# EugenHotaj/pytorch-generative

Measured on AMD Instinct MI355X. Metric: training images/sec (ImageGPT 8-block/4-head/16-embed, 28x28x1), higher is better.
Workload: dtype f32; 1 GPU; BASELINE.json configs[1]: ImageGPT 8 blocks / 4 heads / 16 embed on 28x28x1 binarised-MNIST-shaped synthetic; one step = zero_grad + fwd + BCE + bwd + global grad-norm + Adam + lr decay (reference trainer.py:173-193); per_gpu_batch=1024, global_batch=1024, parallelism=dp1, launch=hipGraph replay

## Files before the change

### include/pg_hip.h

```cpp
#ifndef PG_HIP_H_
#define PG_HIP_H_

#include <stddef.h>
#include <stdint.h>

#ifdef __cplusplus
extern "C" {
#endif

#define PG_ABI_VERSION 2

#define PG_EINVAL (-1)
#define PG_ESHAPE (-2)

#define PG_MAX_TAPS 64

#define PG_ACT_NONE 0
#define PG_ACT_RELU 1
#define PG_ACT_ELU 2
#define PG_ACT_GELU 3
#define PG_ACT_ELU_OUT 4

#define PG_GATE_TANH 0
#define PG_GATE_IDENTITY 1

int pg_abi_version(void);
const char* pg_last_error(void);

int pg_conv2d_taps(const float* in, const float* wpk, const float* bias, const float* res,
                   float* out, int N, int Cin, int IH, int IW, int Cout, int OH, int OW,
                   int T, const int* tap_dr, const int* tap_dc, int in_act,
                   const float* dact_src, int dact, void* stream);

int pg_pack_conv_weight(const float* w, float* wpk, int Cout, int Cin, int KH, int KW, int T,
                        const int* tap_u, const int* tap_v, int transpose, int b_pad,
                        void* stream);
size_t pg_packed_weight_floats(int a, int T, int b);
int pg_conv_b_pad(int b);

int pg_conv2d_mfma(const float* in, const float* wfrag, const float* bias, const float* res,
                   float* out, int N, int Cin, int IH, int IW, int Cout, int OH, int OW, int T,
                   const int* tap_dr, const int* tap_dc, int in_act, const float* dact_src,
                   int dact, int out_act, int fmt, void* stream);
int pg_conv2d_mfma_ex(const float* in, const float* wfrag, const float* bias, const float* res,
                      float* out, int N, int Cin, int IH, int IW, int Cout, int OH, int OW, int T,
                      const int* tap_dr, const int* tap_dc, int in_act, const float* dact_src,
                      int dact, int out_act, int fmt, const float* res2, long res_bs, long res2_bs,
                      void* stream);
int pg_conv_gate_fusable(int Cin, int Cout, int OH, int OW, int T, const int* tap_dr, const int* tap_dc);
int pg_conv2d_mfma_gate(const float* in, const float* wfrag, const float* bias, const float* res, float* out, int N, int Cin,
                        int IH, int IW, int Cout, int OH, int OW, int T, const int* tap_dr, const int* tap_dc, int in_act, int gate,
                        const float* gate_res, float* gate_out, void* stream);
int pg_conv_dual_ok(int Cin, int Cout, int OH, int OW);
int pg_conv2d_mfma_dual(const float* in, const float* wfrag, float* out, float* out2, int N, int Cin, int OH, int OW, int Cout,
                        const float* dact_src, int dact, const float* r, void* stream);
#define PG_CONV_FMT_F32 1
#define PG_CONV_FMT_B3 2
#define PG_CONV_FMT_B3_GATE 3
int pg_conv_mfma_supported(int Cin, int Cout, int T, int OH, int OW, int IW, int hr, int hc);
size_t pg_conv_frag_floats(int K_channels, int M_channels, int T, int fmt);
int pg_pack_conv_weight_frag(const float* w, float* wfrag, int Cout, int Cin, int KH, int KW,
                             int T, const int* tap_u, const int* tap_v, int transpose, int fmt,
                             void* stream);
int pg_pack_conv_weight_frag2(const float* w, float* wfrag_fwd, float* wfrag_dgrad, int Cout,
                              int Cin, int KH, int KW, int T, const int* tap_u, const int* tap_v,
                              int fmt_fwd, int fmt_dgrad, void* stream);

int pg_conv2d_wgrad(const float* x, const float* dy, float* dw, float* db, int N, int Cin,
                    int IH, int IW, int Cout, int OH, int OW, int KH, int KW, int T,
                    const int* tap_dr, const int* tap_dc, const int* tap_u, const int* tap_v,
                    int in_act, float* workspace, size_t workspace_floats, void* stream);
size_t pg_conv2d_wgrad_workspace_floats(int Cout, int Cin, int T);

int pg_mul_inplace(float* w, const float* mask, size_t n, void* stream);

int pg_nchw_layernorm_fwd(const float* x, const float* gamma, const float* beta, float* y,
                          float* mean, float* rstd, int N, int C, int L, float eps,
                          void* stream);
int pg_nchw_layernorm_bwd(const float* x, const float* gamma, const float* mean,
                          const float* rstd, const float* dy, float* dx, float* dgamma,
                          float* dbeta, int N, int C, int L, float* workspace,
                          size_t workspace_floats, void* stream);
size_t pg_nchw_layernorm_bwd_workspace_floats(int N, int C, int L);
int pg_nchw_layernorm_bwd_res(const float* x, const float* gamma, const float* mean,
                              const float* rstd, const float* dy, const float* dx_add, float* dx,
                              float* dgamma, float* dbeta, int N, int C, int L, float* workspace,
                              size_t workspace_floats, void* stream);

int pg_causal_attn_fwd(const float* q, const float* k, const float* v, float* o, float* lse2,
                       int N, int heads, int L, int dk, int dv, long q_bs, long k_bs, long v_bs,
                       long o_bs, int strict, void* stream);
int pg_causal_attn_bwd(const float* q, const float* k, const float* v, const float* o,
                       const float* d_o, const float* lse2, float* delta, float* dq, float* dk,
                       float* dv, int N, int heads, int L, int dk_dim, int dv_dim, long q_bs,
                       long k_bs, long v_bs, long o_bs, long do_bs, long dq_bs, long dk_bs,
                       long dv_bs, int strict, void* stream);

int pg_causal_attn_bwd_dq(const float* q, const float* k, const float* v, const float* o,
                          const float* d_o, const float* lse2, float* delta, float* dq, float* dk,
                          float* dv, int N, int heads, int L, int dk_dim, int dv_dim, long q_bs,
                          long k_bs, long v_bs, long o_bs, long do_bs, long dq_bs, long dk_bs,
                          long dv_bs, int strict, void* stream);
int pg_causal_attn_bwd_dkv(const float* q, const float* k, const float* v, const float* o,
                           const float* d_o, const float* lse2, float* delta, float* dq, float* dk,
                           float* dv, int N, int heads, int L, int dk_dim, int dv_dim, long q_bs,
                           long k_bs, long v_bs, long o_bs, long do_bs, long dq_bs, long dk_bs,
                           long dv_bs, int strict, void* stream);

int pg_attn_fused_bwd(int enable);

int pg_attn_block_plan(int which, int L, int waves, int* out_blk, int* out_q0, int* out_ngrp, int* out_wave,
                       int* out_cost);

#define PG_FEATURE_IDENTITY 0
#define PG_FEATURE_ELU1 1
size_t pg_linear_attn_workspace_floats(int N, int heads, int L, int dk, int dv, int backward);
int pg_linear_attn_fwd(const float* q, const float* k, const float* v, float* out, float* den, float* ws,
                       size_t ws_floats, int N, int heads, int L, int dk, int dv, long q_bs, long kv_bs,
                       long o_bs, int feature, void* stream);
int pg_linear_attn_bwd(const float* q, const float* k, const float* v, const float* out, const float* den,
                       const float* g, float* dq, float* dk, float* dv, float* ws, size_t ws_floats, int N,
                       int heads, int L, int dk_dim, int dv_dim, long q_bs, long kv_bs, long o_bs, int feature,
                       void* stream);

size_t pg_masked_linear_workspace_floats(int N, int in, int out, int dgrad);
int pg_masked_linear_fwd(const float* x, float* w, const float* b, const int* deg_in, const int* deg_out, int strict,
                         float* y, int N, int in, int out, int relu, float* ws, size_t ws_floats, void* stream);
int pg_masked_linear_dgrad(const float* dy, const float* w, const int* deg_in, const int* deg_out, int strict,
                           const float* relu_out, float* dx, int N, int in, int out, float* ws, size_t ws_floats,
                           void* stream);
int pg_masked_linear_wgrad(const float* x, const float* dy, float* dw, float* db, int N, int in, int out,
                           void* stream);
int pg_masked_linear_mask(float* mask, const int* deg_in, const int* deg_out, int strict, int in, int out,
                          void* stream);

#define PG_MIXTURE_BERNOULLI 0
#define PG_MIXTURE_GAUSSIAN 1
size_t pg_mixture_workspace_floats(int kind, int N, int K, int F, int backward);
int pg_mixture_fwd(int kind, const float* x, const float* mixture_logits, const float* p1, const float* p2, float* lse,
                   float* stats, int N, int K, int F, float* ws, size_t ws_floats, void* stream);
int pg_mixture_bwd(int kind, const float* x, const float* mixture_logits, const float* p1, const float* p2,
                   const float* stats, const float* g, float* d_logits, float* d1, float* d2, int N, int K, int F,
                   float* ws, size_t ws_floats, void* stream);
size_t pg_kde_workspace_floats(int N, int K, int F);
int pg_kde_gaussian(const float* test, const float* train, float bandwidth, float* out, int N, int K, int F, float* ws,
                    size_t ws_floats, void* stream);
int pg_kde_parzen(const float* test, const float* train, float bandwidth, float coef, float* out, int N, int K, int F,
                  void* stream);

int pg_image_positional_encoding(float* out, int N, int H, int W, void* stream);

int pg_act_fwd(const float* x, float* y, size_t n, int act, void* stream);
int pg_act_bwd(const float* x, const float* dy, float* dx, size_t n, int act, void* stream);
int pg_gated_fwd(const float* x, float* y, int N, int C, int L, int gate, void* stream);
int pg_gated_bwd(const float* x, const float* dy, float* dx, int N, int C, int L, int gate,
                 void* stream);
int pg_gated_fwd_res(const float* x, const float* res, float* y, int N, int C, int L, int gate,
                     void* stream);
int pg_act_bwd_from_out(const float* y, const float* res, const float* dy, float* dx, size_t n,
                        int act, void* stream);
int pg_add(const float* a, const float* b, float* out, size_t n, void* stream);
int pg_fill(float* out, float value, size_t n, void* stream);
int pg_sum_rows(const float* const* rows, const long* batch_strides, int n_rows, float* out, long n_batch, long per, void* stream);
int pg_add_bcast_fwd(const float* x, const float* p, float* y, int N, size_t per, void* stream);
int pg_add_bcast_bwd(const float* dy, float* dp, int N, size_t per, void* stream);

int pg_bce_logits_fwd(const float* z, const float* x, float* loss, int N, size_t per,
                      void* stream);
int pg_bce_logits_bwd(const float* z, const float* x, const float* gscale, float* dz, int N,
                      size_t per, void* stream);

int pg_avgpool2_fwd(const float* x, float* y, int planes, int OH, int OW, void* stream);
int pg_avgpool2_bwd(const float* dy, float* dx, int planes, int OH, int OW, void* stream);
int pg_avgpool2_bwd_res(const float* dy, const float* res, float* dx, int planes, int OH, int OW, void* stream);
int pg_upsample2_fwd(const float* x, float* y, int planes, int IH, int IW, void* stream);
int pg_upsample2_bwd(const float* dy, float* dx, int planes, int IH, int IW, void* stream);
int pg_phase_split2(float* x, float* xs, int planes, int H, int W, int merge, void* stream);
int pg_phase_merge4(float* x, float* const* p, int planes, int H, int W, int merge, void* stream);
int pg_phase_weights(const float* w, float* out, int A, int B, int transposed, void* stream);
int pg_phase_weights_bwd(const float* const* g, float* dw, int A, int B, int transposed, int accumulate, void* stream);
int pg_gauss_head_fwd(const float* q, const float* p, const float* eps, float* z, float* kl, int N,
                      int C, int L, long q_bs, long p_bs, int mode, void* stream);
int pg_gauss_head_bwd(const float* q, const float* p, const float* eps, const float* dz,
                      const float* dkl, float* dq, float* dp, int N, int C, int L, long q_bs,
                      long p_bs, int mode, void* stream);
int pg_vec_mean_accum(const float* v, int n, float* out, void* stream);
int pg_fill_scaled(const float* g, float scale, float* out, int n, void* stream);

int pg_mlp_gelu_fwd(const float* x, const float* w1, const float* b1, const float* w2,
                    const float* b2, const float* res, float* y, int N, int C, int Hd, int L,
                    void* stream);
int pg_mlp_gelu_bwd(const float* x, const float* w1, const float* b1, const float* w2,
                    const float* dy, float* dx, float* dw1, float* db1, float* dw2, float* db2,
                    int N, int C, int Hd, int L, float* workspace, size_t workspace_floats,
                    void* stream);
size_t pg_mlp_gelu_bwd_workspace_floats(int N, int L);

int pg_gpt_block_head_fwd(const float* x, const float* ln_w, const float* ln_b, const float* wq,
                          const float* bq, const float* wkv, const float* bkv, float* qkv, int N,
                          int C, int L, float eps, void* stream);
int pg_gpt_block_head_bwd(const float* x, const float* ln_w, const float* ln_b, const float* wq,
                          const float* wkv, const float* dqkv, const float* gx, float* dx,
                          float* dln_w, float* dln_b, float* dwq, float* dbq, float* dwkv,
                          float* dbkv, int N, int C, int L, float eps, float* workspace,
                          size_t workspace_floats, void* stream);
size_t pg_gpt_block_head_bwd_workspace_floats(int N, int L);
int pg_gpt_block_tail_fwd(const float* o, const float* x, const float* wp, const float* bp,
                          const float* ln_w, const float* ln_b, const float* w1, const float* b1,
                          const float* w2, const float* b2, float* x_new, int N, int C, int Hd,
                          int L, float eps, void* stream);
int pg_gpt_block_tail_bwd(const float* o, const float* x, const float* wp, const float* bp,
                          const float* ln_w, const float* ln_b, const float* w1, const float* b1,
                          const float* w2, const float* dx_new, float* d_o, float* gx, float* dwp,
                          float* dbp, float* dln_w, float* dln_b, float* dw1, float* db1,
                          float* dw2, float* db2, int N, int C, int Hd, int L, float eps,
                          float* workspace, size_t workspace_floats, void* stream);
size_t pg_gpt_block_tail_bwd_workspace_floats(int N, int L);
int pg_gpt_block_tail_bwd_partial(const float* o, const float* x, const float* wp, const float* bp,
                                  const float* ln_w, const float* ln_b, const float* w1, const float* b1,
                                  const float* w2, const float* dx_new, float* d_o, float* gx, int N, int Cc,
                                  int Hd, int L, float eps, float* workspace, size_t workspace_floats,
                                  void* stream);
int pg_gpt_block_head_bwd_with_tail(const float* x, const float* ln_w, const float* ln_b, const float* wq,
                                    const float* wkv, const float* dqkv, const float* gx, float* dx,
                                    float* dln_w, float* dln_b, float* dwq, float* dbq, float* dwkv,
                                    float* dbkv, int N, int Cc, int L, float eps, float* workspace,
                                    size_t workspace_floats, const float* tail_workspace, float* t_dw1,
                                    float* t_db1, float* t_dw2, float* t_db2, float* t_dwp, float* t_dbp,
                                    float* t_dln_w, float* t_dln_b, void* stream);
int pg_gpt_block_head_bwd_partial(const float* x, const float* ln_w, const float* ln_b, const float* wq, const float* wkv,
                                  const float* dqkv, const float* gx, float* dx, int N, int C, int L, float eps,
                                  float* workspace, size_t workspace_floats, void* stream);
int pg_gpt_blocks_reduce(int n_blocks, const float* const* head_ws, const float* const* tail_ws, float* const* grads,
                         int N, int C, int L, void* stream);

int pg_sample_embed(const float* canvas, const float* pos, const float* w, const float* b, float* out,
                    int N, int Cin, int H, int W, int Cout, int KH, int KW, int r, int c, int ld,
                    const int* pos_dev, void* stream);
int pg_attn_decode(const float* qkv, float* k_cache, float* v_cache, float* o, int N, int heads,
                   int L, int p, int dk, int dv, int ld, int strict, const int* pos_dev,
                   void* stream);

int pg_sumsq_accum(const float* g, size_t n, float* state, void* stream);
int pg_adam_prepare(float* state, void* stream);
int pg_sumsq_partial_count(size_t n);
int pg_sumsq_partials(const float* g, size_t n, float* partials, void* stream);
int pg_adam_prepare_ordered(float* state, const float* partials, int nparts, void* stream);
int pg_adam_step(float* p, const float* g, float* m, float* v, size_t n, const float* state,
                 float beta1, float beta2, float eps, void* stream);

int pg_vq_assign(const float* x, const float* embedding, int* idx, float* q, float* st, float* loss,
                 int N, int D, int L, int K, void* stream);
int pg_vq_ema_update(const float* x, const int* idx, float* cluster_size, float* embedding_avg,
                     float* embedding, float* count_ws, float* sum_ws, int N, int D, int L, int K,
                     float decay, void* stream);
int pg_vq_bwd(const float* x, const float* q, const float* d_st, const float* g_loss, float* dx,
              size_t n, void* stream);
int pg_vq_assign_tiled(const float* x, const float* embedding, int* idx, float* q, float* st, float* loss,
                       int N, int D, int L, int K, void* stream);
size_t pg_vq_codebook_grad_workspace_floats(int N, int D, int L, int K);
int pg_vq_codebook_grad(const float* x, const float* q, const int* idx, const float* g_loss, float* d_embedding,
                        int accumulate, int N, int D, int L, int K, float* ws, size_t ws_floats, void* stream);
int pg_mse_fwd(const float* a, const float* b, float* loss, size_t n, void* stream);
int pg_mse_bwd(const float* a, const float* b, const float* g_loss, float* da, float* db, size_t n,
               void* stream);

int pg_concat_elu_fwd(const float* x, float* y, int N, long CL, void* stream);
int pg_concat_elu_bwd(const float* x, const float* dy, float* dx, int N, long CL, void* stream);

int pg_dmol_fwd(const float* l, const float* x, float* loss, int N, int K, int L, void* stream);
int pg_dmol_bwd(const float* l, const float* x, const float* gscale, float* dl, int N, int K, int L,
                void* stream);

#define PG_DMOL_SAMPLE_MAX_K 32
int pg_dmol_sample(const float* params, long sp_n, long sp_c, long sp_w, const float* uniforms, float* canvas,
                   const unsigned char* unknown, float* row_buf, int N, int K, int H, int W, int r, int c,
                   const int* pos_dev, void* stream);

int pg_col_subsample2(const float* x, float* y, long rows, int W, void* stream);
int pg_col_zero_insert2(const float* x, float* y, long rows, int W, void* stream);

int pg_copy_rows(const float* src, float* dst, long rows, long row_len, long src_stride,
                 long dst_stride, int accumulate, void* stream);

#define PG_COMM_ID_BYTES 128
#define PG_DTYPE_F32 0
int pg_comm_unique_id(char id[PG_COMM_ID_BYTES]);
int pg_comm_init(int rank, int world, const char id[PG_COMM_ID_BYTES]);
int pg_comm_world(void);
int pg_comm_rccl_version(void);
int pg_allreduce_sum(void* buf, size_t n, int dtype, void* stream);
int pg_broadcast(void* buf, size_t n, int dtype, int root, void* stream);
int pg_comm_destroy(void);

#ifdef __cplusplus
}
#endif
#endif
```

### pytorch-generative_amd/csrc/gpt_block.hip

```cpp
#include <stdlib.h>

#include "common.h"

namespace {

typedef float f32x4 __attribute__((ext_vector_type(4)));
#define MFMA16(A, B, C) __builtin_amdgcn_mfma_f32_16x16x4f32((A), (B), (C), 0, 0, 0)

constexpr int C = 16, HD = 64, QKV = 48;
constexpr int GB_THREADS = 256;
constexpr int TS = 20;
constexpr float INV_C = 1.f / 16.f;

constexpr int TB_WAVE_ROWS = 2 * HD + 4 * C;
constexpr int T_W1 = 0, T_B1 = T_W1 + HD * C, T_W2 = T_B1 + HD, T_B2 = T_W2 + C * HD, T_WP = T_B2 + C,
              T_BP = T_WP + C * C, T_G2 = T_BP + C, T_BE2 = T_G2 + C, T_PART = T_BE2 + C;
constexpr int H_WQ = 0, H_WKV = H_WQ + C * C, H_BQ = H_WKV + 2 * C * C, H_BKV = H_BQ + C,
              H_G1 = H_BKV + 2 * C, H_BE1 = H_G1 + C, H_PART = H_BE1 + C;

struct BlockArgs {
  const float* x; const float* g1; const float* be1; const float* wq; const float* bq;
  const float* wkv; const float* bkv; float* qkv; const float* dqkv; const float* gx; float* dx;
  const float* o; const float* wp; const float* bp; const float* g2; const float* be2;
  const float* w1; const float* b1; const float* w2; const float* b2;
  float* xnew; const float* dxnew; float* d_o; float* gx_out;
  float* part;
  int N, L, tiles_per_img, total_tiles;
  float eps;
};

struct Ln { float mu, rs; f32x4 xhat; };

__device__ __forceinline__ float gsum4(float s) {
  s += __shfl_xor(s, 16, 64);
  s += __shfl_xor(s, 32, 64);
  return s;
}
__device__ __forceinline__ float jsum16(float s) {
  s += __shfl_xor(s, 1, 64); s += __shfl_xor(s, 2, 64); s += __shfl_xor(s, 4, 64); s += __shfl_xor(s, 8, 64);
  return s;
}

__device__ __forceinline__ Ln ln_stats(const f32x4& v, float eps) {
  Ln s;
  s.mu = gsum4((v[0] + v[1]) + (v[2] + v[3])) * INV_C;
  const f32x4 dd = {v[0] - s.mu, v[1] - s.mu, v[2] - s.mu, v[3] - s.mu};
  const float a = gsum4(fmaf(dd[0], dd[0], fmaf(dd[1], dd[1], fmaf(dd[2], dd[2], dd[3] * dd[3])))) * INV_C + eps;
  float rs = rsqrtf(a);
  rs = rs * (1.5f - 0.5f * a * rs * rs);
  s.rs = rs;
  s.xhat = f32x4{dd[0] * rs, dd[1] * rs, dd[2] * rs, dd[3] * rs};
  return s;
}

__device__ __forceinline__ f32x4 load_tile(const float* __restrict__ base, int L, int g) {
  f32x4 t;
#pragma unroll
  for (int r = 0; r < 4; ++r) t[r] = base[(size_t)(4 * g + r) * L];
  return t;
}
__device__ __forceinline__ void store_tile(float* __restrict__ base, int L, int g, const f32x4& t) {
#pragma unroll
  for (int r = 0; r < 4; ++r) base[(size_t)(4 * g + r) * L] = t[r];
}
__device__ __forceinline__ f32x4 load_vec(const float* __restrict__ v, int g) {
  return f32x4{v[4 * g], v[4 * g + 1], v[4 * g + 2], v[4 * g + 3]};
}

__device__ __forceinline__ float gelu_f(float x) { return pg_gelu(x); }

struct TileWalk {
  int n, t, dn, dt, tpi;
  __device__ __forceinline__ TileWalk(const BlockArgs& a, int wave, int nwaves)
      : n(wave / a.tiles_per_img), t(wave % a.tiles_per_img), dn(nwaves / a.tiles_per_img),
        dt(nwaves % a.tiles_per_img), tpi(a.tiles_per_img) {}
  __device__ __forceinline__ TileWalk next() const {
    TileWalk w = *this;
    w.n += dn; w.t += dt;
    if (w.t >= tpi) { w.t -= tpi; ++w.n; }
    return w;
  }
  __device__ __forceinline__ size_t base(int chans, int L) const { return ((size_t)n * chans) * L + t * 16; }
};
__device__ __forceinline__ void prefetch_fence() { __builtin_amdgcn_sched_barrier(0); }
constexpr int waitcnt_gfx9(int vm, int exp, int lgkm) { return ((vm & 0x30) << 10) | (vm & 0xF) | ((exp & 7) << 4) | ((lgkm & 0xF) << 8); }
#if defined(__HIP_DEVICE_COMPILE__) && !defined(__GFX9__)
#error "wait_prologue_loads() encodes s_waitcnt for gfx9; re-derive the immediate for another target"
#endif
__device__ __forceinline__ void wait_prologue_loads() {
  constexpr int VMCNT0_ONLY = waitcnt_gfx9( 0,  7,  15);
  static_assert(VMCNT0_ONLY == 0x0F70, "gfx9 s_waitcnt vmcnt(0)");
  __builtin_amdgcn_s_waitcnt(VMCNT0_ONLY);
}
__device__ __forceinline__ void lds_put_tile(float* t, int j, int g, const f32x4& v) {
#pragma unroll
  for (int r = 0; r < 4; ++r) t[(4 * g + r) * TS + j] = v[r];
}
__device__ __forceinline__ f32x4 lds_row4(const float* t, int row, int g) {
  return *reinterpret_cast<const f32x4*>(t + row * TS + 4 * g);
}

__device__ __forceinline__ const float* qkv_row(const BlockArgs& a, int ch) {
  return ch < C ? a.wq + ch * C : a.wkv + (ch - C) * C;
}

__global__ void __launch_bounds__(GB_THREADS) head_fwd_kernel(const BlockArgs a) {
  const int lane = threadIdx.x & 63, j = lane & 15, g = lane >> 4;
  const int wave = blockIdx.x * (GB_THREADS / 64) + __builtin_amdgcn_readfirstlane(threadIdx.x >> 6);
  const int nwaves = gridDim.x * (GB_THREADS / 64);
  float wf[3][4];
  f32x4 bias[3];
#pragma unroll
  for (int m = 0; m < 3; ++m) {
#pragma unroll
    for (int r = 0; r < 4; ++r) {
      wf[m][r] = qkv_row(a, 16 * m + j)[4 * g + r];
      const int ch = 16 * m + 4 * g + r;
      bias[m][r] = ch < C ? a.bq[ch] : a.bkv[ch - C];
    }
  }
  const f32x4 gam = load_vec(a.g1, g), bet = load_vec(a.be1, g);
  if (wave >= a.total_tiles) return;
  TileWalk tw(a, wave, nwaves);
  f32x4 xv = load_tile(a.x + tw.base(C, a.L) + j, a.L, g);
  wait_prologue_loads();
  for (;;) {
    const TileWalk nx = tw.next();
    const bool more = nx.n < a.N;
    const f32x4 xn = load_tile(a.x + (more ? nx : tw).base(C, a.L) + j, a.L, g);
    prefetch_fence();
    const Ln s = ln_stats(xv, a.eps);
    f32x4 y;
#pragma unroll
    for (int r = 0; r < 4; ++r) y[r] = fmaf(s.xhat[r], gam[r], bet[r]);
    float* qb = a.qkv + tw.base(QKV, a.L) + j;
#pragma unroll
    for (int m = 0; m < 3; ++m) {
      f32x4 out = bias[m];
#pragma unroll
      for (int r = 0; r < 4; ++r) out = MFMA16(wf[m][r], y[r], out);
      store_tile(qb + (size_t)(16 * m) * a.L, a.L, g, out);
    }
    if (!more) break;
    xv = xn;
    tw = nx;
  }
}

__global__ void __launch_bounds__(GB_THREADS) head_bwd_kernel(const BlockArgs a) {
  extern __shared__ float4 lds4[];
  float* lds = reinterpret_cast<float*>(lds4);
  const int lane = threadIdx.x & 63, j = lane & 15, g = lane >> 4;
  const int wv = __builtin_amdgcn_readfirstlane(threadIdx.x >> 6);
  const int wave = blockIdx.x * (GB_THREADS / 64) + wv;
  const int nwaves = gridDim.x * (GB_THREADS / 64);
  float* ty = lds + (size_t)wv * (C + QKV) * TS;
  float* tq = ty + C * TS;

  float wt[3][4];
#pragma unroll
  for (int m = 0; m < 3; ++m) {
#pragma unroll
    for (int r = 0; r < 4; ++r) wt[m][r] = qkv_row(a, 16 * m + 4 * g + r)[j];
  }
  const f32x4 gam = load_vec(a.g1, g), bet = load_vec(a.be1, g);
  const f32x4 zero4 = {0.f, 0.f, 0.f, 0.f};
  f32x4 accw[3], accb[3], dgam = zero4, dbet = zero4;
#pragma unroll
  for (int m = 0; m < 3; ++m) { accw[m] = zero4; accb[m] = zero4; }

  if (wave < a.total_tiles) {
    TileWalk tw(a, wave, nwaves);
    size_t off = tw.base(C, a.L) + j;
    f32x4 xv = load_tile(a.x + off, a.L, g);
    f32x4 gxv = load_tile(a.gx + off, a.L, g);
    wait_prologue_loads();
    for (;;) {
      f32x4 dqv[3];
      {
        const float* dqp = a.dqkv + tw.base(QKV, a.L) + j;
#pragma unroll
        for (int m = 0; m < 3; ++m) dqv[m] = load_tile(dqp + (size_t)(16 * m) * a.L, a.L, g);
      }
      const TileWalk nx = tw.next();
      const bool more = nx.n < a.N;
      const size_t offn = (more ? nx : tw).base(C, a.L) + j;
      const f32x4 xn = load_tile(a.x + offn, a.L, g);
      const f32x4 gxn = load_tile(a.gx + offn, a.L, g);
      prefetch_fence();
#pragma unroll
      for (int m = 0; m < 3; ++m) lds_put_tile(tq + 16 * m * TS, j, g, dqv[m]);
      const Ln s = ln_stats(xv, a.eps);
      f32x4 dy = zero4;
#pragma unroll
      for (int m = 0; m < 3; ++m) {
#pragma unroll
        for (int r = 0; r < 4; ++r) {
          dy = MFMA16(wt[m][r], dqv[m][r], dy);
          accb[m][r] += dqv[m][r];
        }
      }
      f32x4 gy;
      float s1 = 0.f, s2 = 0.f;
#pragma unroll
      for (int r = 0; r < 4; ++r) {
        gy[r] = dy[r] * gam[r];
        s1 += gy[r];
        s2 = fmaf(gy[r], s.xhat[r], s2);
        dgam[r] = fmaf(dy[r], s.xhat[r], dgam[r]);
        dbet[r] += dy[r];
        ty[(4 * g + r) * TS + j] = fmaf(s.xhat[r], gam[r], bet[r]);
      }
      const float m1 = gsum4(s1) * INV_C, m2 = gsum4(s2) * INV_C;
      f32x4 dxv;
#pragma unroll
      for (int r = 0; r < 4; ++r) dxv[r] = s.rs * (gy[r] - m1 - s.xhat[r] * m2) + gxv[r];
      store_tile(a.dx + off, a.L, g, dxv);
      const f32x4 yt = lds_row4(ty, j, g);
#pragma unroll
      for (int m = 0; m < 3; ++m) {
        const f32x4 dqtm = lds_row4(tq, 16 * m + j, g);
#pragma unroll
        for (int e = 0; e < 4; ++e) accw[m] = MFMA16(dqtm[e], yt[e], accw[m]);
      }
      if (!more) break;
      xv = xn;
      gxv = gxn;
      off = offn;
      tw = nx;
    }
  }

  __syncthreads();
  float* mine = lds + (size_t)wv * H_PART;
#pragma unroll
  for (int m = 0; m < 3; ++m) {
#pragma unroll
    for (int r = 0; r < 4; ++r) {
      const int ch = 16 * m + 4 * g + r;
      mine[H_WQ + ch * C + j] = accw[m][r];
      const float b = jsum16(accb[m][r]);
      if (j == 0) mine[H_BQ + ch] = b;
    }
  }
#pragma unroll
  for (int r = 0; r < 4; ++r) {
    const float dg = jsum16(dgam[r]), db = jsum16(dbet[r]);
    if (j == 0) { mine[H_G1 + 4 * g + r] = dg; mine[H_BE1 + 4 * g + r] = db; }
  }
  __syncthreads();
  float* prow = a.part + (size_t)blockIdx.x * H_PART;
  for (int i = threadIdx.x; i < H_PART; i += GB_THREADS)
    prow[i] = (lds[i] + lds[H_PART + i]) + (lds[2 * H_PART + i] + lds[3 * H_PART + i]);
}

__global__ void __launch_bounds__(GB_THREADS) tail_fwd_kernel(const BlockArgs a) {
  const int lane = threadIdx.x & 63, j = lane & 15, g = lane >> 4;
  const int wave = blockIdx.x * (GB_THREADS / 64) + __builtin_amdgcn_readfirstlane(threadIdx.x >> 6);
  const int nwaves = gridDim.x * (GB_THREADS / 64);
  float wpf[4], w1f[4][4], w2f[4][4];
  f32x4 b1r[4];
#pragma unroll
  for (int r = 0; r < 4; ++r) wpf[r] = a.wp[j * C + 4 * g + r];
#pragma unroll
  for (int m = 0; m < 4; ++m) {
#pragma unroll
    for (int r = 0; r < 4; ++r) {
      w1f[m][r] = a.w1[(16 * m + j) * C + 4 * g + r];
      w2f[m][r] = a.w2[j * HD + 16 * m + 4 * g + r];
      b1r[m][r] = a.b1[16 * m + 4 * g + r];
    }
  }
  const f32x4 bpv = load_vec(a.bp, g), b2v = load_vec(a.b2, g);
  const f32x4 gam = load_vec(a.g2, g), bet = load_vec(a.be2, g);
  if (wave >= a.total_tiles) return;
  TileWalk tw(a, wave, nwaves);
  size_t off = tw.base(C, a.L) + j;
  f32x4 xv = load_tile(a.x + off, a.L, g);
  f32x4 ov = load_tile(a.o + off, a.L, g);
  wait_prologue_loads();
  for (;;) {
    const TileWalk nx = tw.next();
    const bool more = nx.n < a.N;
    const size_t offn = (more ? nx : tw).base(C, a.L) + j;
    const f32x4 xn = load_tile(a.x + offn, a.L, g);
    const f32x4 on = load_tile(a.o + offn, a.L, g);
    prefetch_fence();
    f32x4 xm = xv + bpv;
#pragma unroll
    for (int r = 0; r < 4; ++r) xm = MFMA16(wpf[r], ov[r], xm);
    const Ln s = ln_stats(xm, a.eps);
    f32x4 y;
#pragma unroll
    for (int r = 0; r < 4; ++r) y[r] = fmaf(s.xhat[r], gam[r], bet[r]);
    f32x4 h[4];
#pragma unroll
    for (int m = 0; m < 4; ++m) {
      h[m] = b1r[m];
#pragma unroll
      for (int r = 0; r < 4; ++r) h[m] = MFMA16(w1f[m][r], y[r], h[m]);
    }
    f32x4 out = (xm + b2v) + xv;
#pragma unroll
    for (int m = 0; m < 4; ++m) {
#pragma unroll
      for (int r = 0; r < 4; ++r) out = MFMA16(w2f[m][r], gelu_f(h[m][r]), out);
    }
    store_tile(a.xnew + off, a.L, g, out);
    if (!more) break;
    xv = xn;
    ov = on;
    off = offn;
    tw = nx;
  }
}

__global__ void __launch_bounds__(GB_THREADS) tail_bwd_kernel(const BlockArgs a) {
  extern __shared__ float4 lds4[];
  float* lds = reinterpret_cast<float*>(lds4);
  const int lane = threadIdx.x & 63, j = lane & 15, g = lane >> 4;
  const int wv = __builtin_amdgcn_readfirstlane(threadIdx.x >> 6);
  const int wave = blockIdx.x * (GB_THREADS / 64) + wv;
  const int nwaves = gridDim.x * (GB_THREADS / 64);
  float* tg = lds + (size_t)wv * TB_WAVE_ROWS * TS;
  float* th = tg + HD * TS;
  float* ty = th + HD * TS;
  float* tx = ty + C * TS;
  float* td = tx + C * TS;
  float* to = td + C * TS;

  float* wl = lds + (size_t)4 * TB_WAVE_ROWS * TS;
  if (wv == 0) {
#pragma unroll
    for (int m = 0; m < 4; ++m) {
#pragma unroll
      for (int r = 0; r < 4; ++r) {
        wl[(0 + 4 * m + r) * 64 + lane] = a.w1[(16 * m + j) * C + 4 * g + r];
        wl[(16 + 4 * m + r) * 64 + lane] = a.w2[(4 * g + r) * HD + 16 * m + j];
        wl[(32 + 4 * m + r) * 64 + lane] = a.w1[(16 * m + 4 * g + r) * C + j];
        wl[(48 + 4 * m + r) * 64 + lane] = a.b1[16 * m + 4 * g + r];
      }
    }
  }
  __syncthreads();
  const float* wlane = wl + lane;
#define W1F(m, r) wlane[(0 + 4 * (m) + (r)) * 64]
#define W2T(m, r) wlane[(16 + 4 * (m) + (r)) * 64]
#define W1T(m, r) wlane[(32 + 4 * (m) + (r)) * 64]
#define B1R(m, r) wlane[(48 + 4 * (m) + (r)) * 64]
  float wpf[4], wpt[4];
#pragma unroll
  for (int r = 0; r < 4; ++r) {
    wpf[r] = a.wp[j * C + 4 * g + r];
    wpt[r] = a.wp[(4 * g + r) * C + j];
  }
  const f32x4 bpv = load_vec(a.bp, g);
  const f32x4 gam = load_vec(a.g2, g), bet = load_vec(a.be2, g);
  const f32x4 zero4 = {0.f, 0.f, 0.f, 0.f};
  f32x4 acc1[4], acc2[4], db1[4], accp = zero4, db2 = zero4, dbp = zero4, dgam = zero4, dbet = zero4;
#pragma unroll
  for (int m = 0; m < 4; ++m) { acc1[m] = zero4; acc2[m] = zero4; db1[m] = zero4; }

  if (wave < a.total_tiles) {
    TileWalk tw(a, wave, nwaves);
    size_t off = tw.base(C, a.L) + j;
    f32x4 xv = load_tile(a.x + off, a.L, g);
    f32x4 ov = load_tile(a.o + off, a.L, g);
    f32x4 dv = load_tile(a.dxnew + off, a.L, g);
    wait_prologue_loads();
    for (;;) {
      const TileWalk nx = tw.next();
      const bool more = nx.n < a.N;
      const size_t offn = (more ? nx : tw).base(C, a.L) + j;
      const f32x4 xn = load_tile(a.x + offn, a.L, g);
      const f32x4 on = load_tile(a.o + offn, a.L, g);
      const f32x4 dn = load_tile(a.dxnew + offn, a.L, g);
      prefetch_fence();
      lds_put_tile(td, j, g, dv);
      lds_put_tile(to, j, g, ov);

      f32x4 xm = xv + bpv;
#pragma unroll
      for (int r = 0; r < 4; ++r) xm = MFMA16(wpf[r], ov[r], xm);
      const Ln s = ln_stats(xm, a.eps);
      f32x4 y;
#pragma unroll
      for (int r = 0; r < 4; ++r) {
        y[r] = fmaf(s.xhat[r], gam[r], bet[r]);
        ty[(4 * g + r) * TS + j] = y[r];
        db2[r] += dv[r];
      }
      f32x4 h[4], dg[4];
#pragma unroll
      for (int m = 0; m < 4; ++m) {
        h[m] = f32x4{B1R(m, 0), B1R(m, 1), B1R(m, 2), B1R(m, 3)};
        dg[m] = zero4;
#pragma unroll
        for (int r = 0; r < 4; ++r) {
          h[m] = MFMA16(W1F(m, r), y[r], h[m]);
          dg[m] = MFMA16(W2T(m, r), dv[r], dg[m]);
        }
      }
      f32x4 dy = zero4;
#pragma unroll
      for (int m = 0; m < 4; ++m) {
#pragma unroll
        for (int r = 0; r < 4; ++r) {
          const float hv = h[m][r];
          float cdf, ee;
          pg_gelu_parts(hv, cdf, ee);
          const float pdf = 0.39894228040143267794f * ee;
          const float dh = dg[m][r] * (cdf + hv * pdf);
          const int hid = 16 * m + 4 * g + r;
          tg[hid * TS + j] = hv * cdf;
          th[hid * TS + j] = dh;
          db1[m][r] += dh;
          dy = MFMA16(W1T(m, r), dh, dy);
        }
      }
      f32x4 gy, dxm;
      float s1 = 0.f, s2 = 0.f;
#pragma unroll
      for (int r = 0; r < 4; ++r) {
        gy[r] = dy[r] * gam[r];
        s1 += gy[r];
        s2 = fmaf(gy[r], s.xhat[r], s2);
        dgam[r] = fmaf(dy[r], s.xhat[r], dgam[r]);
        dbet[r] += dy[r];
      }
      const float m1 = gsum4(s1) * INV_C, m2 = gsum4(s2) * INV_C;
      f32x4 dov = zero4, gxv;
#pragma unroll
      for (int r = 0; r < 4; ++r) {
        dxm[r] = dv[r] + s.rs * (gy[r] - m1 - s.xhat[r] * m2);
        tx[(4 * g + r) * TS + j] = dxm[r];
        dbp[r] += dxm[r];
        gxv[r] = dv[r] + dxm[r];
      }
#pragma unroll
      for (int r = 0; r < 4; ++r) dov = MFMA16(wpt[r], dxm[r], dov);
      store_tile(a.d_o + off, a.L, g, dov);
      store_tile(a.gx_out + off, a.L, g, gxv);

      const f32x4 yt = lds_row4(ty, j, g);
      const f32x4 xt = lds_row4(tx, j, g);
      const f32x4 dvt = lds_row4(td, j, g);
      const f32x4 ot = lds_row4(to, j, g);
#pragma unroll
      for (int e = 0; e < 4; ++e) accp = MFMA16(xt[e], ot[e], accp);
#pragma unroll
      for (int m = 0; m < 4; ++m) {
        const f32x4 gt = *reinterpret_cast<const f32x4*>(tg + (16 * m + j) * TS + 4 * g);
        const f32x4 ht = *reinterpret_cast<const f32x4*>(th + (16 * m + j) * TS + 4 * g);
#pragma unroll
        for (int e = 0; e < 4; ++e) {
          acc2[m] = MFMA16(dvt[e], gt[e], acc2[m]);
          acc1[m] = MFMA16(ht[e], yt[e], acc1[m]);
        }
      }
      if (!more) break;
      xv = xn;
      ov = on;
      dv = dn;
      off = offn;
      tw = nx;
    }
  }

#undef W1F
#undef W2T
#undef W1T
#undef B1R
  __syncthreads();
  float* mine = lds + (size_t)wv * T_PART;
#pragma unroll
  for (int m = 0; m < 4; ++m) {
#pragma unroll
    for (int r = 0; r < 4; ++r) {
      mine[T_W1 + (16 * m + 4 * g + r) * C + j] = acc1[m][r];
      mine[T_W2 + (4 * g + r) * HD + 16 * m + j] = acc2[m][r];
      const float v = jsum16(db1[m][r]);
      if (j == 0) mine[T_B1 + 16 * m + 4 * g + r] = v;
    }
  }
#pragma unroll
  for (int r = 0; r < 4; ++r) {
    mine[T_WP + (4 * g + r) * C + j] = accp[r];
    const float v2 = jsum16(db2[r]), vp = jsum16(dbp[r]), vg = jsum16(dgam[r]), vb = jsum16(dbet[r]);
    if (j == 0) {
      mine[T_B2 + 4 * g + r] = v2;
      mine[T_BP + 4 * g + r] = vp;
      mine[T_G2 + 4 * g + r] = vg;
      mine[T_BE2 + 4 * g + r] = vb;
    }
  }
  __syncthreads();
  float* prow = a.part + (size_t)blockIdx.x * T_PART;
  for (int i = threadIdx.x; i < T_PART; i += GB_THREADS)
    prow[i] = (lds[i] + lds[T_PART + i]) + (lds[2 * T_PART + i] + lds[3 * T_PART + i]);
}

struct SegArgs {
  const float* part; int rows, stride, nseg;
  int end[8]; float* dst[8];
};
__global__ void __launch_bounds__(256) seg_reduce_kernel(const SegArgs a) {
  __shared__ float red[32][9];
  const int sl = threadIdx.x & 7, rg = threadIdx.x >> 3;
  const int s = blockIdx.x * 8 + sl;
  float a0 = 0.f, a1 = 0.f;
  if (s < a.stride) {
    const float* p = a.part + s;
    int r = rg;
    for (; r + 32 < a.rows; r += 64) {
      a0 += p[(size_t)r * a.stride];
      a1 += p[(size_t)(r + 32) * a.stride];
    }
    if (r < a.rows) a0 += p[(size_t)r * a.stride];
  }
  red[rg][sl] = a0 + a1;
  __syncthreads();
  if (rg != 0 || s >= a.stride) return;
  float acc = 0.f;
#pragma unroll
  for (int r = 0; r < 32; ++r) acc += red[r][sl];
  int begin = 0;
  for (int k = 0; k < a.nseg; ++k) {
    if (s < a.end[k]) { a.dst[k][s - begin] += acc; return; }
    begin = a.end[k];
  }
}

struct SegArgs2 { SegArgs j[2]; int blocks0; };
__global__ void __launch_bounds__(256) seg_reduce2_kernel(const SegArgs2 a2) {
  __shared__ float red[32][9];
  const bool second = (int)blockIdx.x >= a2.blocks0;
  const SegArgs& a = a2.j[second ? 1 : 0];
  const int blk = second ? blockIdx.x - a2.blocks0 : blockIdx.x;
  const int sl = threadIdx.x & 7, rg = threadIdx.x >> 3;
  const int s = blk * 8 + sl;
  float a0 = 0.f, a1 = 0.f;
  if (s < a.stride) {
    const float* p = a.part + s;
    int r = rg;
    for (; r + 32 < a.rows; r += 64) {
      a0 += p[(size_t)r * a.stride];
      a1 += p[(size_t)(r + 32) * a.stride];
    }
    if (r < a.rows) a0 += p[(size_t)r * a.stride];
  }
  red[rg][sl] = a0 + a1;
  __syncthreads();
  if (rg != 0 || s >= a.stride) return;
  float acc = 0.f;
#pragma unroll
  for (int r = 0; r < 32; ++r) acc += red[r][sl];
  int begin = 0;
  for (int k = 0; k < a.nseg; ++k) {
    if (s < a.end[k]) { a.dst[k][s - begin] += acc; return; }
    begin = a.end[k];
  }
}

constexpr int SEG_MAX_JOBS = 16;
struct SegArgsN { SegArgs j[SEG_MAX_JOBS]; int first[SEG_MAX_JOBS + 1]; int n; };
__global__ void __launch_bounds__(256) seg_reduceN_kernel(const SegArgsN an) {
  __shared__ float red[32][9];
  int job = 0;
  while (job + 1 < an.n && (int)blockIdx.x >= an.first[job + 1]) ++job;
  const SegArgs& a = an.j[job];
  const int blk = blockIdx.x - an.first[job];
  const int sl = threadIdx.x & 7, rg = threadIdx.x >> 3;
  const int s = blk * 8 + sl;
  float a0 = 0.f, a1 = 0.f;
  if (s < a.stride) {
    const float* p = a.part + s;
    int r = rg;
    for (; r + 32 < a.rows; r += 64) {
      a0 += p[(size_t)r * a.stride];
      a1 += p[(size_t)(r + 32) * a.stride];
    }
    if (r < a.rows) a0 += p[(size_t)r * a.stride];
  }
  red[rg][sl] = a0 + a1;
  __syncthreads();
  if (rg != 0 || s >= a.stride) return;
  float acc = 0.f;
#pragma unroll
  for (int r = 0; r < 32; ++r) acc += red[r][sl];
  int begin = 0;
  for (int k = 0; k < a.nseg; ++k) {
    if (s < a.end[k]) { a.dst[k][s - begin] += acc; return; }
    begin = a.end[k];
  }
}

int grid_blocks(int which, int N, int L) {
  struct Cfg { int cap[4]; int mt[2]; };
  static const Cfg cfg = []() {
    Cfg c = {{2048, 1024, 2048, 512},
             {1, 2}};
    if (const char* e = PG_AB_ENV("PG_BLOCK_GRID")) {
      int v[4];
      if (sscanf(e, "%d,%d,%d,%d", &v[0], &v[1], &v[2], &v[3]) == 4 && v[0] > 0 && v[1] > 0 && v[2] > 0 && v[3] > 0)
        for (int i = 0; i < 4; ++i) c.cap[i] = v[i];
    }
    if (const char* e = PG_AB_ENV("PG_BLOCK_MINTILES")) {
      int f = 0, b = 0;
      if (sscanf(e, "%d,%d", &f, &b) == 2 && f > 0 && b > 0) { c.mt[0] = f; c.mt[1] = b; }
    }
    return c;
  }();
  const int* cap = cfg.cap;
  const int* mt_cfg = cfg.mt;
  const int min_tiles = (which & 1) ? mt_cfg[1] : mt_cfg[0];
  const long tiles = (long)N * (L / 16);
  long b = (tiles + 4 * min_tiles - 1) / (4 * min_tiles);
  if (b > cap[which]) b = cap[which];
  return b < 1 ? 1 : (int)b;
}
int bwd_blocks(int N, int L) { return grid_blocks(3, N, L); }

int check_shape(const char* who, int N, int Cc, int L) {
  PG_REQUIRE(N > 0 && L > 0, PG_EINVAL, "%s: non-positive dimension", who);
  PG_REQUIRE(Cc == C, PG_ESHAPE, "%s: only C = 16 is instantiated (got %d)", who, Cc);
  PG_REQUIRE(L % 16 == 0, PG_ESHAPE, "%s: L=%d is not a multiple of 16", who, L);
  return 0;
}

void set_geometry(BlockArgs& a, int N, int L, float eps) {
  a.N = N; a.L = L; a.tiles_per_img = L / 16; a.total_tiles = N * a.tiles_per_img; a.eps = eps;
}

bool al16(const void* p) { return (reinterpret_cast<uintptr_t>(p) & 15) == 0; }

}

PG_EXPORT size_t pg_gpt_block_head_bwd_workspace_floats(int N, int L) {
  if (N <= 0 || L < 16) return 0;
  return (size_t)grid_blocks(1, N, L) * H_PART;
}
PG_EXPORT size_t pg_gpt_block_tail_bwd_workspace_floats(int N, int L) {
  if (N <= 0 || L < 16) return 0;
  return (size_t)grid_blocks(3, N, L) * T_PART;
}

PG_EXPORT int pg_gpt_block_head_fwd(const float* x, const float* ln_w, const float* ln_b, const float* wq,
                                    const float* bq, const float* wkv, const float* bkv, float* qkv,
                                    int N, int Cc, int L, float eps, void* stream) {
  PG_REQUIRE(x && ln_w && ln_b && wq && bq && wkv && bkv && qkv, PG_EINVAL, "pg_gpt_block_head_fwd: null pointer");
  int rc = check_shape("pg_gpt_block_head_fwd", N, Cc, L);
  if (rc) return rc;
  BlockArgs a = {};
  a.x = x; a.g1 = ln_w; a.be1 = ln_b; a.wq = wq; a.bq = bq; a.wkv = wkv; a.bkv = bkv; a.qkv = qkv;
  set_geometry(a, N, L, eps);
  hipLaunchKernelGGL(head_fwd_kernel, dim3((unsigned)grid_blocks(0, N, L)), dim3(GB_THREADS), 0, (hipStream_t)stream, a);
  PG_LAUNCH_CHECK("pg_gpt_block_head_fwd");
  return 0;
}

namespace {
SegArgs tail_seg_args(const float* workspace, int rows, float* dw1, float* db1, float* dw2, float* db2,
                      float* dwp, float* dbp, float* dln_w, float* dln_b) {
  SegArgs r = {};
  r.part = workspace; r.rows = rows; r.stride = T_PART; r.nseg = 8;
  r.end[0] = T_B1; r.dst[0] = dw1;
  r.end[1] = T_W2; r.dst[1] = db1;
  r.end[2] = T_B2; r.dst[2] = dw2;
  r.end[3] = T_WP; r.dst[3] = db2;
  r.end[4] = T_BP; r.dst[4] = dwp;
  r.end[5] = T_G2; r.dst[5] = dbp;
  r.end[6] = T_BE2; r.dst[6] = dln_w;
  r.end[7] = T_PART; r.dst[7] = dln_b;
  return r;
}

SegArgs head_seg_args(const float* workspace, int rows, float* dln_w, float* dln_b, float* dwq, float* dbq, float* dwkv,
                      float* dbkv) {
  SegArgs r = {};
  r.part = workspace; r.rows = rows; r.stride = H_PART; r.nseg = 6;
  r.end[0] = H_WKV; r.dst[0] = dwq;
  r.end[1] = H_BQ; r.dst[1] = dwkv;
  r.end[2] = H_BKV; r.dst[2] = dbq;
  r.end[3] = H_G1; r.dst[3] = dbkv;
  r.end[4] = H_BE1; r.dst[4] = dln_w;
  r.end[5] = H_PART; r.dst[5] = dln_b;
  return r;
}

int head_bwd_impl(const float* x, const float* ln_w, const float* ln_b, const float* wq, const float* wkv,
                  const float* dqkv, const float* gx, float* dx, float* dln_w, float* dln_b, float* dwq,
                  float* dbq, float* dwkv, float* dbkv, int N, int Cc, int L, float eps, float* workspace,
                  size_t workspace_floats, const SegArgs* tail, void* stream, int defer = 0) {
  PG_REQUIRE(x && ln_w && ln_b && wq && wkv && dqkv && gx && dx && workspace &&
                 (defer || (dln_w && dln_b && dwq && dbq && dwkv && dbkv)), PG_EINVAL, "pg_gpt_block_head_bwd: null pointer");
  int rc = check_shape("pg_gpt_block_head_bwd", N, Cc, L);
  if (rc) return rc;
  PG_REQUIRE(workspace_floats >= pg_gpt_block_head_bwd_workspace_floats(N, L), PG_EINVAL,
             "pg_gpt_block_head_bwd: workspace too small");
  PG_REQUIRE(al16(dqkv), PG_EINVAL, "pg_gpt_block_head_bwd: dqkv must be 16-byte aligned");
  BlockArgs a = {};
  a.x = x; a.g1 = ln_w; a.be1 = ln_b; a.wq = wq; a.wkv = wkv; a.dqkv = dqkv; a.gx = gx; a.dx = dx;
  a.part = workspace;
  set_geometry(a, N, L, eps);
  const int blocks = grid_blocks(1, N, L);
  hipStream_t st = (hipStream_t)stream;
  const size_t tr = (size_t)4 * (C + QKV) * TS, rd = (size_t)4 * H_PART;
  hipLaunchKernelGGL(head_bwd_kernel, dim3((unsigned)blocks), dim3(GB_THREADS), (tr > rd ? tr : rd) * sizeof(float), st, a);
  PG_LAUNCH_CHECK("pg_gpt_block_head_bwd");
  if (defer) return 0;
  const SegArgs r = head_seg_args(workspace, blocks, dln_w, dln_b, dwq, dbq, dwkv, dbkv);
  if (tail) {
    SegArgs2 r2;
    r2.j[0] = r; r2.j[1] = *tail; r2.blocks0 = (H_PART + 7) / 8;
    hipLaunchKernelGGL(seg_reduce2_kernel, dim3((unsigned)(r2.blocks0 + (T_PART + 7) / 8)), dim3(256), 0, st, r2);
  } else {
    hipLaunchKernelGGL(seg_reduce_kernel, dim3((unsigned)((H_PART + 7) / 8)), dim3(256), 0, st, r);
  }
  PG_LAUNCH_CHECK("pg_gpt_block_head_bwd(reduce)");
  return 0;
}
}

PG_EXPORT int pg_gpt_block_head_bwd(const float* x, const float* ln_w, const float* ln_b, const float* wq,
                                    const float* wkv, const float* dqkv, const float* gx, float* dx,
                                    float* dln_w, float* dln_b, float* dwq, float* dbq, float* dwkv,
                                    float* dbkv, int N, int Cc, int L, float eps, float* workspace,
                                    size_t workspace_floats, void* stream) {
  return head_bwd_impl(x, ln_w, ln_b, wq, wkv, dqkv, gx, dx, dln_w, dln_b, dwq, dbq, dwkv, dbkv, N, Cc, L, eps,
                       workspace, workspace_floats, nullptr, stream);
}

PG_EXPORT int pg_gpt_block_head_bwd_with_tail(const float* x, const float* ln_w, const float* ln_b, const float* wq,
                                              const float* wkv, const float* dqkv, const float* gx, float* dx,
                                              float* dln_w, float* dln_b, float* dwq, float* dbq, float* dwkv,
                                              float* dbkv, int N, int Cc, int L, float eps, float* workspace,
                                              size_t workspace_floats, const float* tail_workspace, float* t_dw1,
                                              float* t_db1, float* t_dw2, float* t_db2, float* t_dwp, float* t_dbp,
                                              float* t_dln_w, float* t_dln_b, void* stream) {
  PG_REQUIRE(tail_workspace && t_dw1 && t_db1 && t_dw2 && t_db2 && t_dwp && t_dbp && t_dln_w && t_dln_b, PG_EINVAL,
             "pg_gpt_block_head_bwd_with_tail: null pointer");
  if (int rc = check_shape("pg_gpt_block_head_bwd_with_tail", N, Cc, L)) return rc;
  const SegArgs tail = tail_seg_args(tail_workspace, bwd_blocks(N, L), t_dw1, t_db1, t_dw2, t_db2, t_dwp, t_dbp,
                                     t_dln_w, t_dln_b);
  return head_bwd_impl(x, ln_w, ln_b, wq, wkv, dqkv, gx, dx, dln_w, dln_b, dwq, dbq, dwkv, dbkv, N, Cc, L, eps,
                       workspace, workspace_floats, &tail, stream);
}

PG_EXPORT int pg_gpt_block_head_bwd_partial(const float* x, const float* ln_w, const float* ln_b, const float* wq,
                                            const float* wkv, const float* dqkv, const float* gx, float* dx, int N, int Cc,
                                            int L, float eps, float* workspace, size_t workspace_floats, void* stream) {
  return head_bwd_impl(x, ln_w, ln_b, wq, wkv, dqkv, gx, dx, nullptr, nullptr, nullptr, nullptr, nullptr, nullptr, N, Cc, L,
                       eps, workspace, workspace_floats, nullptr, stream, 1);
}

PG_EXPORT int pg_gpt_blocks_reduce(int n_blocks, const float* const* head_ws, const float* const* tail_ws, float* const* grads,
                                   int N, int Cc, int L, void* stream) {
  PG_REQUIRE(head_ws && tail_ws && grads, PG_EINVAL, "pg_gpt_blocks_reduce: null pointer");
  PG_REQUIRE(n_blocks >= 1 && 2 * n_blocks <= SEG_MAX_JOBS, PG_ESHAPE, "pg_gpt_blocks_reduce: 1..8 blocks per launch, got %d", n_blocks);
  if (int rc = check_shape("pg_gpt_blocks_reduce", N, Cc, L)) return rc;
  SegArgsN an = {};
  int nb = 0;
  for (int b = 0; b < n_blocks; ++b) {
    float* const* g = grads + 14 * b;
    PG_REQUIRE(head_ws[b] && tail_ws[b], PG_EINVAL, "pg_gpt_blocks_reduce: null workspace of block %d", b);
    for (int k = 0; k < 14; ++k) PG_REQUIRE(g[k], PG_EINVAL, "pg_gpt_blocks_reduce: null gradient %d of block %d", k, b);
    an.j[2 * b] = head_seg_args(head_ws[b], grid_blocks(1, N, L), g[0], g[1], g[2], g[3], g[4], g[5]);
    an.first[2 * b] = nb; nb += (H_PART + 7) / 8;
    an.j[2 * b + 1] = tail_seg_args(tail_ws[b], bwd_blocks(N, L), g[6], g[7], g[8], g[9], g[10], g[11], g[12], g[13]);
    an.first[2 * b + 1] = nb; nb += (T_PART + 7) / 8;
  }
  an.n = 2 * n_blocks;
  an.first[an.n] = nb;
  hipLaunchKernelGGL(seg_reduceN_kernel, dim3((unsigned)nb), dim3(256), 0, (hipStream_t)stream, an);
  PG_LAUNCH_CHECK("pg_gpt_blocks_reduce");
  return 0;
}

PG_EXPORT int pg_gpt_block_tail_fwd(const float* o, const float* x, const float* wp, const float* bp,
                                    const float* ln_w, const float* ln_b, const float* w1, const float* b1,
                                    const float* w2, const float* b2, float* x_new, int N, int Cc, int Hd,
                                    int L, float eps, void* stream) {
  PG_REQUIRE(o && x && wp && bp && ln_w && ln_b && w1 && b1 && w2 && b2 && x_new, PG_EINVAL,
             "pg_gpt_block_tail_fwd: null pointer");
  int rc = check_shape("pg_gpt_block_tail_fwd", N, Cc, L);
  if (rc) return rc;
  PG_REQUIRE(Hd == HD, PG_ESHAPE, "pg_gpt_block_tail_fwd: only hidden = 64 is instantiated (got %d)", Hd);
  BlockArgs a = {};
  a.o = o; a.x = x; a.wp = wp; a.bp = bp; a.g2 = ln_w; a.be2 = ln_b; a.w1 = w1; a.b1 = b1; a.w2 = w2;
  a.b2 = b2; a.xnew = x_new;
  set_geometry(a, N, L, eps);
  hipLaunchKernelGGL(tail_fwd_kernel, dim3((unsigned)grid_blocks(2, N, L)), dim3(GB_THREADS), 0, (hipStream_t)stream, a);
  PG_LAUNCH_CHECK("pg_gpt_block_tail_fwd");
  return 0;
}

namespace {
int tail_bwd_impl(const float* o, const float* x, const float* wp, const float* bp,
                                    const float* ln_w, const float* ln_b, const float* w1, const float* b1,
                                    const float* w2, const float* dx_new, float* d_o, float* gx,
                                    float* dwp, float* dbp, float* dln_w, float* dln_b, float* dw1,
                                    float* db1, float* dw2, float* db2, int N, int Cc, int Hd, int L,
                                    float eps, float* workspace, size_t workspace_floats, bool reduce_now, void* stream) {
  PG_REQUIRE(o && x && wp && bp && ln_w && ln_b && w1 && b1 && w2 && dx_new && d_o && gx && dwp && dbp &&
                 dln_w && dln_b && dw1 && db1 && dw2 && db2 && workspace, PG_EINVAL,
             "pg_gpt_block_tail_bwd: null pointer");
  int rc = check_shape("pg_gpt_block_tail_bwd", N, Cc, L);
  if (rc) return rc;
  PG_REQUIRE(Hd == HD, PG_ESHAPE, "pg_gpt_block_tail_bwd: only hidden = 64 is instantiated (got %d)", Hd);
  PG_REQUIRE(workspace_floats >= pg_gpt_block_tail_bwd_workspace_floats(N, L), PG_EINVAL,
             "pg_gpt_block_tail_bwd: workspace too small");
  PG_REQUIRE(al16(o) && al16(dx_new), PG_EINVAL, "pg_gpt_block_tail_bwd: o / dx_new must be 16-byte aligned");
  BlockArgs a = {};
  a.o = o; a.x = x; a.wp = wp; a.bp = bp; a.g2 = ln_w; a.be2 = ln_b; a.w1 = w1; a.b1 = b1; a.w2 = w2;
  a.dxnew = dx_new; a.d_o = d_o; a.gx_out = gx; a.part = workspace;
  set_geometry(a, N, L, eps);
  const int blocks = bwd_blocks(N, L);
  hipStream_t st = (hipStream_t)stream;
  const size_t tr = (size_t)4 * TB_WAVE_ROWS * TS + 64 * 64, rd = (size_t)4 * T_PART;
  const size_t shmem = (tr > rd ? tr : rd) * sizeof(float);
  static const hipError_t attr = hipFuncSetAttribute(reinterpret_cast<const void*>(tail_bwd_kernel),
                                                     hipFuncAttributeMaxDynamicSharedMemorySize, 80 * 1024);
  (void)attr;
  hipLaunchKernelGGL(tail_bwd_kernel, dim3((unsigned)blocks), dim3(GB_THREADS), shmem, st, a);
  PG_LAUNCH_CHECK("pg_gpt_block_tail_bwd");
  if (!reduce_now) return 0;
  const SegArgs r = tail_seg_args(workspace, blocks, dw1, db1, dw2, db2, dwp, dbp, dln_w, dln_b);
  hipLaunchKernelGGL(seg_reduce_kernel, dim3((unsigned)((T_PART + 7) / 8)), dim3(256), 0, st, r);
  PG_LAUNCH_CHECK("pg_gpt_block_tail_bwd(reduce)");
  return 0;
}
}

PG_EXPORT int pg_gpt_block_tail_bwd(const float* o, const float* x, const float* wp, const float* bp,
                                    const float* ln_w, const float* ln_b, const float* w1, const float* b1,
                                    const float* w2, const float* dx_new, float* d_o, float* gx,
                                    float* dwp, float* dbp, float* dln_w, float* dln_b, float* dw1,
                                    float* db1, float* dw2, float* db2, int N, int Cc, int Hd, int L,
                                    float eps, float* workspace, size_t workspace_floats, void* stream) {
  return tail_bwd_impl(o, x, wp, bp, ln_w, ln_b, w1, b1, w2, dx_new, d_o, gx, dwp, dbp, dln_w, dln_b, dw1, db1, dw2,
                       db2, N, Cc, Hd, L, eps, workspace, workspace_floats, true, stream);
}

PG_EXPORT int pg_gpt_block_tail_bwd_partial(const float* o, const float* x, const float* wp, const float* bp,
                                            const float* ln_w, const float* ln_b, const float* w1, const float* b1,
                                            const float* w2, const float* dx_new, float* d_o, float* gx, int N,
                                            int Cc, int Hd, int L, float eps, float* workspace,
                                            size_t workspace_floats, void* stream) {
  float* dummy = workspace;
  return tail_bwd_impl(o, x, wp, bp, ln_w, ln_b, w1, b1, w2, dx_new, d_o, gx, dummy, dummy, dummy, dummy, dummy, dummy,
                       dummy, dummy, N, Cc, Hd, L, eps, workspace, workspace_floats, false, stream);
}
```

### pytorch-generative_amd/pytorch_generative_amd/_lib.py

```python

import ctypes
import os

_HERE = os.path.dirname(os.path.abspath(__file__))
LIB_PATH = os.environ.get("PG_HIP_LIB") or os.path.join(_HERE, "lib", "libpg_hip.so")

ABI_VERSION = 2

c_f = ctypes.c_void_p
c_i = ctypes.c_int
c_l = ctypes.c_long
c_z = ctypes.c_size_t
c_s = ctypes.c_void_p
c_ip = ctypes.POINTER(ctypes.c_int)
c_flt = ctypes.c_float

SIGNATURES = {
    "pg_abi_version": (c_i, []),
    "pg_last_error": (ctypes.c_char_p, []),
    "pg_conv2d_taps": (
        c_i,
        [c_f, c_f, c_f, c_f, c_f, c_i, c_i, c_i, c_i, c_i, c_i, c_i, c_i, c_ip, c_ip, c_i, c_f, c_i,
         c_s],
    ),
    "pg_conv2d_mfma": (
        c_i,
        [c_f, c_f, c_f, c_f, c_f, c_i, c_i, c_i, c_i, c_i, c_i, c_i, c_i, c_ip, c_ip, c_i, c_f, c_i,
         c_i, c_i, c_s],
    ),
    "pg_conv2d_mfma_ex": (
        c_i,
        [c_f, c_f, c_f, c_f, c_f, c_i, c_i, c_i, c_i, c_i, c_i, c_i, c_i, c_ip, c_ip, c_i, c_f, c_i,
         c_i, c_i, c_f, c_l, c_l, c_s],
    ),
    "pg_conv_dual_ok": (c_i, [c_i] * 4),
    "pg_conv2d_mfma_dual": (c_i, [c_f] * 4 + [c_i] * 5 + [c_f, c_i, c_f, c_s]),
    "pg_conv_gate_fusable": (c_i, [c_i, c_i, c_i, c_i, c_i, c_ip, c_ip]),
    "pg_conv2d_mfma_gate": (c_i, [c_f, c_f, c_f, c_f, c_f, c_i, c_i, c_i, c_i, c_i, c_i, c_i, c_i, c_ip, c_ip, c_i, c_i, c_f, c_f, c_s]),
    "pg_conv_mfma_supported": (c_i, [c_i, c_i, c_i, c_i, c_i, c_i, c_i, c_i]),
    "pg_conv_frag_floats": (c_z, [c_i, c_i, c_i, c_i]),
    "pg_pack_conv_weight_frag": (c_i, [c_f, c_f, c_i, c_i, c_i, c_i, c_i, c_ip, c_ip, c_i, c_i, c_s]),
    "pg_pack_conv_weight_frag2": (c_i, [c_f, c_f, c_f, c_i, c_i, c_i, c_i, c_i, c_ip, c_ip, c_i, c_i, c_s]),
    "pg_pack_conv_weight": (c_i, [c_f, c_f, c_i, c_i, c_i, c_i, c_i, c_ip, c_ip, c_i, c_i, c_s]),
    "pg_packed_weight_floats": (c_z, [c_i, c_i, c_i]),
    "pg_conv_b_pad": (c_i, [c_i]),
    "pg_conv2d_wgrad": (
        c_i,
        [c_f, c_f, c_f, c_f, c_i, c_i, c_i, c_i, c_i, c_i, c_i, c_i, c_i, c_i, c_ip, c_ip, c_ip,
         c_ip, c_i, c_f, c_z, c_s],
    ),
    "pg_conv2d_wgrad_workspace_floats": (c_z, [c_i, c_i, c_i]),
    "pg_mul_inplace": (c_i, [c_f, c_f, c_z, c_s]),
    "pg_nchw_layernorm_fwd": (c_i, [c_f, c_f, c_f, c_f, c_f, c_f, c_i, c_i, c_i, c_flt, c_s]),
    "pg_nchw_layernorm_bwd": (
        c_i, [c_f, c_f, c_f, c_f, c_f, c_f, c_f, c_f, c_i, c_i, c_i, c_f, c_z, c_s]),
    "pg_gpt_block_head_fwd": (c_i, [c_f] * 8 + [c_i, c_i, c_i, c_flt, c_s]),
    "pg_gpt_block_head_bwd": (c_i, [c_f] * 14 + [c_i, c_i, c_i, c_flt, c_f, c_z, c_s]),
    "pg_gpt_block_head_bwd_workspace_floats": (c_z, [c_i, c_i]),
    "pg_gpt_block_head_bwd_partial": (c_i, [c_f] * 8 + [c_i, c_i, c_i, c_flt, c_f, c_z, c_s]),
    "pg_gpt_blocks_reduce": (c_i, [c_i, ctypes.POINTER(ctypes.c_void_p), ctypes.POINTER(ctypes.c_void_p),
                                   ctypes.POINTER(ctypes.c_void_p), c_i, c_i, c_i, c_s]),
    "pg_gpt_block_tail_fwd": (c_i, [c_f] * 11 + [c_i, c_i, c_i, c_i, c_flt, c_s]),
    "pg_gpt_block_tail_bwd": (c_i, [c_f] * 20 + [c_i, c_i, c_i, c_i, c_flt, c_f, c_z, c_s]),
    "pg_gpt_block_tail_bwd_workspace_floats": (c_z, [c_i, c_i]),
    "pg_gpt_block_tail_bwd_partial": (c_i, [c_f] * 12 + [c_i, c_i, c_i, c_i, c_flt, c_f, c_z, c_s]),
    "pg_gpt_block_head_bwd_with_tail": (c_i, [c_f] * 14 + [c_i, c_i, c_i, c_flt, c_f, c_z] + [c_f] * 9 + [c_s]),
    "pg_sample_embed": (c_i, [c_f] * 5 + [c_i] * 10 + [c_f, c_s]),
    "pg_attn_decode": (c_i, [c_f] * 4 + [c_i] * 8 + [c_f, c_s]),
    "pg_mlp_gelu_fwd": (c_i, [c_f, c_f, c_f, c_f, c_f, c_f, c_f, c_i, c_i, c_i, c_i, c_s]),
    "pg_mlp_gelu_bwd": (
        c_i, [c_f, c_f, c_f, c_f, c_f, c_f, c_f, c_f, c_f, c_f, c_i, c_i, c_i, c_i, c_f, c_z, c_s]),
    "pg_mlp_gelu_bwd_workspace_floats": (c_z, [c_i, c_i]),
    "pg_nchw_layernorm_bwd_res": (
        c_i, [c_f, c_f, c_f, c_f, c_f, c_f, c_f, c_f, c_f, c_i, c_i, c_i, c_f, c_z, c_s]),
    "pg_nchw_layernorm_bwd_workspace_floats": (c_z, [c_i, c_i, c_i]),
    "pg_causal_attn_fwd": (
        c_i,
        [c_f, c_f, c_f, c_f, c_f, c_i, c_i, c_i, c_i, c_i, c_l, c_l, c_l, c_l, c_i, c_s],
    ),
    "pg_causal_attn_bwd": (
        c_i,
        [c_f, c_f, c_f, c_f, c_f, c_f, c_f, c_f, c_f, c_f, c_i, c_i, c_i, c_i, c_i, c_l, c_l, c_l,
         c_l, c_l, c_l, c_l, c_l, c_i, c_s],
    ),
    "pg_causal_attn_bwd_dq": (
        c_i,
        [c_f, c_f, c_f, c_f, c_f, c_f, c_f, c_f, c_f, c_f, c_i, c_i, c_i, c_i, c_i, c_l, c_l, c_l,
         c_l, c_l, c_l, c_l, c_l, c_i, c_s],
    ),
    "pg_causal_attn_bwd_dkv": (
        c_i,
        [c_f, c_f, c_f, c_f, c_f, c_f, c_f, c_f, c_f, c_f, c_i, c_i, c_i, c_i, c_i, c_l, c_l, c_l,
         c_l, c_l, c_l, c_l, c_l, c_i, c_s],
    ),
    "pg_linear_attn_workspace_floats": (c_z, [c_i] * 6),
    "pg_linear_attn_fwd": (c_i, [c_f] * 6 + [c_z] + [c_i] * 5 + [c_l] * 3 + [c_i, c_s]),
    "pg_linear_attn_bwd": (c_i, [c_f] * 10 + [c_z] + [c_i] * 5 + [c_l] * 3 + [c_i, c_s]),
    "pg_masked_linear_workspace_floats": (c_z, [c_i] * 4),
    "pg_masked_linear_fwd": (c_i, [c_f] * 5 + [c_i, c_f] + [c_i] * 4 + [c_f, c_z, c_s]),
    "pg_masked_linear_dgrad": (c_i, [c_f] * 4 + [c_i, c_f, c_f] + [c_i] * 3 + [c_f, c_z, c_s]),
    "pg_masked_linear_wgrad": (c_i, [c_f] * 4 + [c_i] * 3 + [c_s]),
    "pg_masked_linear_mask": (c_i, [c_f] * 3 + [c_i] * 3 + [c_s]),
    "pg_mixture_workspace_floats": (c_z, [c_i] * 5),
    "pg_mixture_fwd": (c_i, [c_i] + [c_f] * 6 + [c_i] * 3 + [c_f, c_z, c_s]),
    "pg_mixture_bwd": (c_i, [c_i] + [c_f] * 9 + [c_i] * 3 + [c_f, c_z, c_s]),
    "pg_kde_workspace_floats": (c_z, [c_i] * 3),
    "pg_kde_gaussian": (c_i, [c_f, c_f, c_flt, c_f] + [c_i] * 3 + [c_f, c_z, c_s]),
    "pg_kde_parzen": (c_i, [c_f, c_f, c_flt, c_flt, c_f] + [c_i] * 3 + [c_s]),
    "pg_image_positional_encoding": (c_i, [c_f, c_i, c_i, c_i, c_s]),
    "pg_act_fwd": (c_i, [c_f, c_f, c_z, c_i, c_s]),
    "pg_act_bwd": (c_i, [c_f, c_f, c_f, c_z, c_i, c_s]),
    "pg_gated_fwd": (c_i, [c_f, c_f, c_i, c_i, c_i, c_i, c_s]),
    "pg_gated_bwd": (c_i, [c_f, c_f, c_f, c_i, c_i, c_i, c_i, c_s]),
    "pg_gated_fwd_res": (c_i, [c_f, c_f, c_f, c_i, c_i, c_i, c_i, c_s]),
    "pg_act_bwd_from_out": (c_i, [c_f, c_f, c_f, c_f, c_z, c_i, c_s]),
    "pg_add": (c_i, [c_f, c_f, c_f, c_z, c_s]),
    "pg_fill": (c_i, [c_f, c_flt, c_z, c_s]),
    "pg_phase_merge4": (c_i, [c_f, ctypes.POINTER(ctypes.c_void_p), c_i, c_i, c_i, c_i, c_s]),
    "pg_phase_weights": (c_i, [c_f, c_f, c_i, c_i, c_i, c_s]),
    "pg_phase_weights_bwd": (c_i, [ctypes.POINTER(ctypes.c_void_p), c_f, c_i, c_i, c_i, c_i, c_s]),
    "pg_sum_rows": (c_i, [ctypes.POINTER(ctypes.c_void_p), ctypes.POINTER(ctypes.c_long), c_i, c_f, c_l, c_l, c_s]),
    "pg_avgpool2_bwd_res": (c_i, [c_f, c_f, c_f, c_i, c_i, c_i, c_s]),
    "pg_add_bcast_fwd": (c_i, [c_f, c_f, c_f, c_i, c_z, c_s]),
    "pg_add_bcast_bwd": (c_i, [c_f, c_f, c_i, c_z, c_s]),
    "pg_vq_assign": (c_i, [c_f, c_f, c_f, c_f, c_f, c_f, c_i, c_i, c_i, c_i, c_s]),
    "pg_vq_ema_update": (c_i, [c_f, c_f, c_f, c_f, c_f, c_f, c_f, c_i, c_i, c_i, c_i, ctypes.c_float, c_s]),
    "pg_vq_bwd": (c_i, [c_f, c_f, c_f, c_f, c_f, c_z, c_s]),
    "pg_vq_assign_tiled": (c_i, [c_f, c_f, c_f, c_f, c_f, c_f, c_i, c_i, c_i, c_i, c_s]),
    "pg_vq_codebook_grad_workspace_floats": (c_z, [c_i, c_i, c_i, c_i]),
    "pg_vq_codebook_grad": (c_i, [c_f, c_f, c_f, c_f, c_f, c_i, c_i, c_i, c_i, c_i, c_f, c_z, c_s]),
    "pg_mse_fwd": (c_i, [c_f, c_f, c_f, c_z, c_s]),
    "pg_mse_bwd": (c_i, [c_f, c_f, c_f, c_f, c_f, c_z, c_s]),
    "pg_bce_logits_fwd": (c_i, [c_f, c_f, c_f, c_i, c_z, c_s]),
    "pg_bce_logits_bwd": (c_i, [c_f, c_f, c_f, c_f, c_i, c_z, c_s]),
    "pg_avgpool2_fwd": (c_i, [c_f, c_f, c_i, c_i, c_i, c_s]),
    "pg_avgpool2_bwd": (c_i, [c_f, c_f, c_i, c_i, c_i, c_s]),
    "pg_upsample2_fwd": (c_i, [c_f, c_f, c_i, c_i, c_i, c_s]),
    "pg_upsample2_bwd": (c_i, [c_f, c_f, c_i, c_i, c_i, c_s]),
    "pg_phase_split2": (c_i, [c_f, c_f, c_i, c_i, c_i, c_i, c_s]),
    "pg_gauss_head_fwd": (c_i, [c_f, c_f, c_f, c_f, c_f, c_i, c_i, c_i, c_l, c_l, c_i, c_s]),
    "pg_gauss_head_bwd": (c_i, [c_f, c_f, c_f, c_f, c_f, c_f, c_f, c_i, c_i, c_i, c_l, c_l, c_i, c_s]),
    "pg_vec_mean_accum": (c_i, [c_f, c_i, c_f, c_s]),
    "pg_fill_scaled": (c_i, [c_f, c_flt, c_f, c_i, c_s]),
    "pg_sumsq_accum": (c_i, [c_f, c_z, c_f, c_s]),
    "pg_adam_prepare": (c_i, [c_f, c_s]),
    "pg_sumsq_partial_count": (c_i, [c_z]),
    "pg_sumsq_partials": (c_i, [c_f, c_z, c_f, c_s]),
    "pg_adam_prepare_ordered": (c_i, [c_f, c_f, c_i, c_s]),
    "pg_adam_step": (c_i, [c_f, c_f, c_f, c_f, c_z, c_f, c_flt, c_flt, c_flt, c_s]),
    "pg_attn_fused_bwd": (c_i, [c_i]),
    "pg_attn_block_plan": (c_i, [c_i, c_i, c_i, c_ip, c_ip, c_ip, c_ip, c_ip]),
    "pg_concat_elu_fwd": (c_i, [c_f, c_f, c_i, c_l, c_s]),
    "pg_concat_elu_bwd": (c_i, [c_f, c_f, c_f, c_i, c_l, c_s]),
    "pg_dmol_fwd": (c_i, [c_f, c_f, c_f, c_i, c_i, c_i, c_s]),
    "pg_dmol_bwd": (c_i, [c_f, c_f, c_f, c_f, c_i, c_i, c_i, c_s]),
    "pg_dmol_sample": (c_i, [c_f, c_l, c_l, c_l, c_f, c_f, c_f, c_f] + [c_i] * 6 + [c_f, c_s]),
    "pg_col_subsample2": (c_i, [c_f, c_f, c_l, c_i, c_s]),
    "pg_col_zero_insert2": (c_i, [c_f, c_f, c_l, c_i, c_s]),
    "pg_copy_rows": (c_i, [c_f, c_f, c_l, c_l, c_l, c_l, c_i, c_s]),
    "pg_comm_unique_id": (c_i, [ctypes.c_char_p]),
    "pg_comm_init": (c_i, [c_i, c_i, ctypes.c_char_p]),
    "pg_comm_world": (c_i, []),
    "pg_comm_rccl_version": (c_i, []),
    "pg_allreduce_sum": (c_i, [c_f, c_z, c_i, c_s]),
    "pg_broadcast": (c_i, [c_f, c_z, c_i, c_i, c_s]),
    "pg_comm_destroy": (c_i, []),
}
COMM_ID_BYTES = 128
DTYPE_F32 = 0

_lib = None


def load():
    global _lib
    if _lib is not None:
        return _lib
    if not os.path.exists(LIB_PATH):
        raise RuntimeError(
            f"libpg_hip.so not found at {LIB_PATH}. Build it with "
            "`python pytorch-generative_amd/build.py` (or __graft_entry__.build()). "
            "There is no CPU/ATen fallback for the HIP operator path."
        )
    lib = ctypes.CDLL(LIB_PATH)
    for name, (restype, argtypes) in SIGNATURES.items():
        fn = getattr(lib, name)
        fn.restype = restype
        fn.argtypes = argtypes
    got = lib.pg_abi_version()
    if got != ABI_VERSION:
        raise RuntimeError(f"libpg_hip.so ABI version {got} != expected {ABI_VERSION}")
    if os.environ.get("PG_TRACE"):
        lib = _Traced(lib, os.environ["PG_TRACE"])
    _lib = lib
    return lib


class _Traced:

    def __init__(self, lib, prefix):
        self._lib = lib
        self._out = open(f"{prefix}.{os.getpid()}", "a", buffering=1)

    def __getattr__(self, name):
        fn = getattr(self._lib, name)
        if not name.startswith("pg_") or name in ("pg_last_error", "pg_abi_version"):
            return fn
        out = self._out

        def call(*args):
            shown = []
            for a in args:
                if isinstance(a, int):
                    shown.append(hex(a) if a > 1 << 32 else str(a))
                elif isinstance(a, ctypes.Array):
                    shown.append(str(list(a)))
                else:
                    shown.append(repr(a))
            out.write(f"{name}({', '.join(shown)})\n")
            return fn(*args)

        setattr(self, name, call)
        return call


def check(rc, what):
    if rc == 0:
        return
    msg = load().pg_last_error().decode("utf-8", "replace")
    if rc < 0:
        raise ValueError(f"{what}: {msg} (status {rc})")
    if rc >= 1000:
        raise RuntimeError(f"{what}: {msg}")
    raise RuntimeError(f"{what}: HIP error {rc}: {msg}")


def int_array(values):
    return (ctypes.c_int * len(values))(*values)
```

### pytorch-generative_amd/pytorch_generative_amd/models/autoregressive/image_gpt.py

```python

import os

import torch
from torch import nn

from pytorch_generative_amd import _lib
from pytorch_generative_amd import nn as pg_nn
from pytorch_generative_amd import ops
from pytorch_generative_amd.models import base

_BLOCK_CHAIN = os.environ.get("PG_BLOCK_CHAIN", "1") != "0"


class TransformerBlock(nn.Module):
    def __init__(self, n_channels, n_attention_heads):
        super().__init__()
        self._ln1 = pg_nn.NCHWLayerNorm(n_channels)
        self._ln2 = pg_nn.NCHWLayerNorm(n_channels)
        self._attn = pg_nn.CausalAttention(
            in_channels=n_channels,
            n_heads=n_attention_heads,
            embed_channels=n_channels,
            out_channels=n_channels,
        )
        self._out = nn.Sequential(
            pg_nn.Conv2d(in_channels=n_channels, out_channels=4 * n_channels, kernel_size=1),
            nn.GELU(),
            pg_nn.Conv2d(in_channels=4 * n_channels, out_channels=n_channels, kernel_size=1),
        )

    def _fused_ok(self, x):
        return ops.gpt_block_supported(x, self._ln1, self._attn._q, self._attn._kv, self._attn._proj,
                                       self._ln2, self._out[0], self._out[2])

    def forward_plus_input(self, x, chain=None, flush=False):
        if not self._fused_ok(x):
            return ops.add(x, self.forward(x))
        attn = self._attn
        pair = {}
        if chain is not None:
            pair["chain"], pair["flush"] = chain, flush
        qkv, xs = ops.gpt_block_head(x, self._ln1, attn._q, attn._kv, pair)
        o = ops.causal_attention_qkv(qkv, attn._n_heads, attn._embed_channels, attn._out_channels,
                                     attn._mask_center)
        return ops.gpt_block_tail(o, xs, attn._proj, self._ln2, self._out[0], self._out[2], pair)

    def forward(self, x):
        y, x = self._ln1(x, skip=True)
        x = self._attn(y, res=x)
        y, x = self._ln2(x, skip=True)
        if ops.mlp_gelu_supported(y, self._out[0], self._out[2]):
            return ops.mlp_gelu(y, self._out[0], self._out[2], res=x)
        hidden = self._out[0](y)
        return self._out[2](hidden, in_act="gelu", res=x)


class ImageGPT(base.AutoregressiveModel):
    def __init__(
        self,
        in_channels=1,
        out_channels=1,
        in_size=28,
        n_transformer_blocks=8,
        n_attention_heads=4,
        n_embedding_channels=16,
        sample_fn=None,
    ):
        super().__init__(sample_fn)
        self._pos = nn.Parameter(torch.zeros(1, in_channels, in_size, in_size))
        self._input = pg_nn.CausalConv2d(
            mask_center=True,
            in_channels=in_channels,
            out_channels=n_embedding_channels,
            kernel_size=3,
            padding=1,
        )
        self._transformer = nn.ModuleList(
            TransformerBlock(n_channels=n_embedding_channels, n_attention_heads=n_attention_heads)
            for _ in range(n_transformer_blocks)
        )
        self._ln = pg_nn.NCHWLayerNorm(n_embedding_channels)
        self._out = pg_nn.Conv2d(
            in_channels=n_embedding_channels, out_channels=out_channels, kernel_size=1
        )

    def _incremental_ok(self, n):
        ld = (n + 15) // 16 * 16
        probe = torch.empty(1, self._input.weight.shape[0], 1, ld, device="meta")
        return all(blk._fused_ok(probe) for blk in self._transformer) and self._input.bias is not None

    @torch.no_grad()
    def sample(self, n_samples=None, conditioned_on=None, *, incremental=True, return_logits=False):
        canvas = self._start_canvas(n_samples, conditioned_on)
        n, c, h, w = canvas.shape
        if not incremental or not self._incremental_ok(n):
            if return_logits:
                raise ValueError("return_logits needs the incremental sampler")
            return super().sample(conditioned_on=canvas)
        lib = _lib.load()
        dev, L = canvas.device, h * w
        canvas = canvas.contiguous()
        ld = (n + 15) // 16 * 16
        conv = self._input
        emb = conv.weight.shape[0]
        kh, kw = conv.weight.shape[2], conv.weight.shape[3]
        ops.mul_inplace_(conv.weight.data, conv.mask)
        blocks = list(self._transformer)
        caches = []
        for blk in blocks:
            a = blk._attn
            caches.append((torch.zeros(n, a._embed_channels, L, device=dev),
                           torch.zeros(n, a._out_channels, L, device=dev)))
        x = torch.zeros(1, emb, 1, ld, device=dev)
        pos_dev = torch.zeros(1, dtype=torch.int32, device=dev)

        def position_logits():
            st = torch.cuda.current_stream().cuda_stream
            _lib.check(lib.pg_sample_embed(canvas.data_ptr(), self._pos.data_ptr(),
                                           conv.weight.data_ptr(), conv.bias.data_ptr(), x.data_ptr(),
                                           n, c, h, w, emb, kh, kw, 0, 0, ld, pos_dev.data_ptr(), st),
                       "pg_sample_embed")
            cur = x
            for blk, (kc, vc) in zip(blocks, caches):
                a = blk._attn
                qkv, xs = ops.gpt_block_head(cur, blk._ln1, a._q, a._kv)
                o = torch.empty(1, a._out_channels, 1, ld, device=dev)
                _lib.check(lib.pg_attn_decode(qkv.data_ptr(), kc.data_ptr(), vc.data_ptr(),
                                              o.data_ptr(), n, a._n_heads, L, 0,
                                              a._embed_channels // a._n_heads,
                                              a._out_channels // a._n_heads, ld, int(a._mask_center),
                                              pos_dev.data_ptr(), st), "pg_attn_decode")
                cur = ops.gpt_block_tail(o, xs, a._proj, blk._ln2, blk._out[0], blk._out[2])
            return self._out(self._ln(cur))[0, :, 0, :n].t().contiguous()

        graph, static_logits = None, None
        try:
            side = torch.cuda.Stream()
            side.wait_stream(torch.cuda.current_stream())
            with torch.cuda.stream(side):
                position_logits()
            torch.cuda.current_stream().wait_stream(side)
            graph = torch.cuda.CUDAGraph()
            with torch.cuda.graph(graph, capture_error_mode="thread_local"):
                static_logits = position_logits()
                pos_dev.add_(1)
        except Exception:
            graph = None
            torch.cuda.synchronize()
        pos_dev.zero_()
        all_logits = []
        for row in range(h):
            for col in range(w):
                if graph is not None:
                    graph.replay()
                    logits = static_logits.clone() if return_logits else static_logits
                else:
                    logits = position_logits()
                    pos_dev.add_(1)
                if return_logits:
                    all_logits.append(logits)
                drawn = self._sample_fn(logits).view(n, c)
                current = canvas[:, :, row, col]
                canvas[:, :, row, col] = torch.where(current < 0, drawn, current)
        if return_logits:
            return canvas, torch.stack(all_logits)
        return canvas

    def forward(self, x):
        x = self._input(ops.add_broadcast_batch(x, self._pos))
        blocks = list(self._transformer)
        chain = None
        if (ops.DEFER_BLOCK_REDUCE and _BLOCK_CHAIN and torch.is_grad_enabled() and x.requires_grad and len(blocks) > 1
                and all(b._fused_ok(x) for b in blocks)):
            chain = ops.new_block_chain()
        for i, block in enumerate(blocks):
            x = block.forward_plus_input(x, chain, flush=(i == 0))
        return self._out(self._ln(x))


def reproduce(n_epochs=457, batch_size=64, log_dir="/tmp/run", n_gpus=1, device_id=0,
              debug_loader=None):
    from pytorch_generative_amd import recipes

    return recipes.run(
        lambda: ImageGPT(in_channels=1, out_channels=1, in_size=28, n_transformer_blocks=8,
                         n_attention_heads=2, n_embedding_channels=64),
        loaders=recipes.binarized_mnist, loss_fn=recipes.bce_loss, lr=5e-3, lr_decay=0.999977,
        n_epochs=n_epochs, batch_size=batch_size, log_dir=log_dir, n_gpus=n_gpus,
        device_id=device_id, debug_loader=debug_loader)
```

### pytorch-generative_amd/pytorch_generative_amd/nn/convolution.py

```python

import torch
from torch import nn

from pytorch_generative_amd import ops

_ACTS = {None: ops.ACT_NONE, "relu": ops.ACT_RELU, "elu": ops.ACT_ELU, "gelu": ops.ACT_GELU}


def _pair(v):
    return tuple(v) if isinstance(v, (tuple, list)) else (v, v)


class Conv2d(nn.Conv2d):

    def __init__(self, *args, **kwargs):
        super().__init__(*args, **kwargs)
        if _pair(self.dilation) != (1, 1) or self.groups != 1:
            raise ValueError("pytorch_generative_amd.nn.Conv2d supports dilation=1, groups=1")
        if self.padding_mode != "zeros" or isinstance(self.padding, str):
            raise ValueError("pytorch_generative_amd.nn.Conv2d supports integer zero padding only")
        self._down2 = False
        if _pair(self.stride) != (1, 1):
            if (_pair(self.stride), _pair(self.kernel_size), _pair(self.padding)) != ((2, 2), (4, 4), (1, 1)):
                raise ValueError(
                    "pytorch_generative_amd.nn.Conv2d supports stride 1, or stride 2 with kernel 4 and padding 1"
                )
            self._down2 = True
        self._spec = None

    def _active_taps(self):
        return None

    def _conv_spec(self):
        if self._spec is None:
            kh, kw = _pair(self.kernel_size)
            ph, pw = _pair(self.padding)
            self._spec = ops.ConvSpec(kh, kw, ph, pw, active=self._active_taps(), wgrad_all=True)
        return self._spec

    def mfma_ok(self, x, crop=None):
        return (not self._down2) and ops.conv_mfma_ok(x, self.weight, self._conv_spec(), crop)

    def _row_reset(self):
        self._row_band = None
        self._row_spec_cached = None

    def _row_forward(self, ctx, x, crop, in_act, res, out_act):
        if self._down2:
            raise ValueError("row decode: strided convolutions are not row-causal")
        spec = self._conv_spec()
        reach = [spec.pad_h - u for u, _ in spec.fwd_taps]
        if min(reach) < 0:
            raise ValueError("row decode: a tap below the output row (the layer is not row-causal)")
        k = max(reach)
        n, c, one, w = x.shape
        if one != 1:
            raise ValueError("row decode expects one image row")
        if getattr(self, "_row_spec_cached", None) is None:
            self._row_spec_cached = ops.ConvSpec(spec.kh, spec.kw, spec.pad_h - k, spec.pad_w,
                                                 active=spec.fwd_taps)
        if k == 0:
            band = x
        else:
            if getattr(self, "_row_band", None) is None or self._row_band.shape != (n, c, k + 1, w):
                self._row_band = torch.zeros((n, c, k + 1, w), device=x.device, dtype=x.dtype)
            band = self._row_band
            band[:, :, k:, :].copy_(x)
        ow = crop[1] if crop is not None else spec.full_out(1, w)[1]
        y = ops.conv2d_taps(band, self.weight, self.bias, self._row_spec_cached, out_hw=(1, ow),
                            in_act=_ACTS[in_act], res=None if out_act is not None else res)
        if out_act is not None:
            y = ops._Act.apply(y, _ACTS[out_act])
            if res is not None:
                y = ops.add(y, res)
        if ctx.commit and k > 0:
            band[:, :, :k, :].copy_(band[:, :, 1:, :].clone())
        return y

    def two_residuals_ok(self, x, crop=None):
        return (not self._down2) and ops.RowDecode.current is None and ops.conv_two_residuals_ok(
            x, self.weight, self._conv_spec(), crop)

    def forward_cat2(self, xa, xb, *, in_act=None, skip_b=False):
        if (self._down2 or ops.RowDecode.current is not None or tuple(self.weight.shape[2:]) != (1, 1)
                or xa.shape[1] + xb.shape[1] != self.weight.shape[1]):
            y = self.forward(torch.cat((xa, xb), dim=1), in_act=in_act)
            return (y, xb) if skip_b else y
        wa, wb = ops.split_in_channels(self.weight, xa.shape[1])
        spec = self._conv_spec()
        h = ops.conv2d_taps(xa, wa, None, spec, in_act=_ACTS[in_act])
        return ops.conv2d_taps(xb, wb, self.bias, spec, in_act=_ACTS[in_act], res=h, bias_param=self.bias,
                               n_skip=1 if skip_b else 0)

    def gate_ok(self, x, crop=None):
        return (not self._down2) and ops.RowDecode.current is None and ops.conv_gate_ok(x, self.weight, self._conv_spec(), crop)

    def dual_ok(self, x, crop=None):
        return ((not self._down2) and ops.RowDecode.current is None and crop is None and self.mfma_ok(x, crop)
                and ops.conv_dual_ok(x, self.weight, self._conv_spec()))

    def forward(self, x, *, crop=None, in_act=None, res=None, out_act=None, out_pre_scaled=False,
                in_post=None, n_skip=0, res2=None, gate=None, gate_res=None, res_slot=None, in_sum=None):
        if res_slot is not None or in_sum is not None:
            if (gate is not None or res2 is not None or n_skip or self._down2 or ops.RowDecode.current is not None
                    or not self.mfma_ok(x, crop)):
                raise ValueError("Conv2d: res_slot / in_sum need the plain matrix-core training path (check dual_ok first)")
            return ops.conv2d_taps(
                x, self.weight, self.bias, self._conv_spec(), out_hw=crop, in_act=_ACTS[in_act],
                res=res, weight_param=self.weight, bias_param=self.bias, out_act=_ACTS[out_act],
                out_pre_scaled=out_pre_scaled, in_post=_ACTS[in_post], res_slot=res_slot, in_sum=in_sum,
            )
        if gate is not None:
            if res2 is not None or out_act is not None or out_pre_scaled or not self.gate_ok(x, crop):
                raise ValueError("Conv2d: gate= needs a convolution (at most one residual) on a shape gate_ok() accepts")
            if n_skip and not x.requires_grad:
                y = ops.conv2d_taps(x, self.weight, self.bias, self._conv_spec(), out_hw=crop, in_act=_ACTS[in_act], res=res,
                                    weight_param=self.weight, bias_param=self.bias, in_post=_ACTS[in_post],
                                    gate=gate, gate_res=gate_res)
                return (y,) + (x,) * n_skip
            return ops.conv2d_taps(x, self.weight, self.bias, self._conv_spec(), out_hw=crop, in_act=_ACTS[in_act], res=res,
                                   weight_param=self.weight, bias_param=self.bias, in_post=_ACTS[in_post], n_skip=n_skip,
                                   gate=gate, gate_res=gate_res)
        if res2 is not None and not self.two_residuals_ok(x, crop):
            y = self.forward(x, crop=crop, in_act=in_act, res=res, out_act=out_act,
                             out_pre_scaled=out_pre_scaled, in_post=in_post, n_skip=n_skip)
            return (ops.add(y[0], res2),) + tuple(y[1:]) if n_skip else ops.add(y, res2)
        if n_skip:
            ctx = ops.RowDecode.current
            if ctx is not None or self._down2 or not x.requires_grad:
                y = self.forward(x, crop=crop, in_act=in_act, res=res, out_act=out_act,
                                 out_pre_scaled=out_pre_scaled, in_post=in_post, res2=res2)
                return (y,) + (x,) * n_skip
        ctx = ops.RowDecode.current
        if ctx is not None:
            return self._row_forward(ctx, x, crop, in_act, res, out_act)
        if self._down2:
            if out_act is not None or in_post is not None:
                raise ValueError("Conv2d: fused output activations are not available for stride 2")
            return self._forward_down2(x, in_act, res)
        if (out_pre_scaled or in_post is not None) and not self.mfma_ok(x, crop):
            raise ValueError("Conv2d: out_pre_scaled / in_post need the matrix-core path for this shape "
                             "(check mfma_ok first)")
        if out_act is not None and not out_pre_scaled and not self.mfma_ok(x, crop):
            y = ops.conv2d_taps(x, self.weight, self.bias, self._conv_spec(), out_hw=crop,
                                in_act=_ACTS[in_act], weight_param=self.weight, bias_param=self.bias)
            y = ops._Act.apply(y, _ACTS[out_act])
            y = y if res is None else ops.add(y, res)
            return (y,) + (x,) * n_skip if n_skip else y
        return ops.conv2d_taps(
            x, self.weight, self.bias, self._conv_spec(), out_hw=crop, in_act=_ACTS[in_act],
            res=res, weight_param=self.weight, bias_param=self.bias, out_act=_ACTS[out_act],
            out_pre_scaled=out_pre_scaled, in_post=_ACTS[in_post], n_skip=n_skip, res2=res2,
        )

    def _forward_down2(self, x, in_act, res):
        xs = ops.phase_split4(x)
        _, _, h, w = xs[0].shape
        out = res
        wph = ops.phase_weights(self.weight)
        for pr in (0, 1):
            for pc in (0, 1):
                wsel = wph[2 * pr + pc]
                spec = _PHASE_SPECS[(pr, pc)]
                last = (pr, pc) == (1, 1)
                out = ops.conv2d_taps(xs[2 * pr + pc], wsel, self.bias if last else None, spec,
                                      out_hw=(h, w), in_act=_ACTS[in_act], res=out)
        return out


_PHASE_SPECS = {
    (pr, pc): ops.ConvSpec(2, 2, pr, pc) for pr in (0, 1) for pc in (0, 1)
}


class ConvTranspose2d(nn.ConvTranspose2d):

    def __init__(self, *args, **kwargs):
        super().__init__(*args, **kwargs)
        ok = (_pair(self.stride), _pair(self.kernel_size), _pair(self.padding)) == ((2, 2), (4, 4), (1, 1))
        if not ok or _pair(self.output_padding) != (0, 0) or self.groups != 1 or _pair(self.dilation) != (1, 1):
            raise ValueError("pytorch_generative_amd.nn.ConvTranspose2d supports kernel 4, stride 2, padding 1")

    def forward(self, x, *, in_act=None):
        wph = ops.phase_weights(self.weight, transposed=True)
        phases = []
        xs = [x] * 4
        for pr in (0, 1):
            for pc in (0, 1):
                k = 2 * pr + pc
                spec = _PHASE_SPECS[(1 - pr, 1 - pc)]
                if k == 0 and x.requires_grad:
                    y, *al = ops.conv2d_taps(x, wph[k], self.bias, spec, out_hw=x.shape[2:], in_act=_ACTS[in_act],
                                             n_skip=3, bias_param=self.bias)
                    xs = [x] + list(al)
                else:
                    y = ops.conv2d_taps(xs[k], wph[k], self.bias, spec, out_hw=x.shape[2:], in_act=_ACTS[in_act],
                                        bias_param=self.bias)
                phases.append(y)
        return ops.phase_merge4(phases)


class CausalConv2d(Conv2d):

    def __init__(self, mask_center, *args, **kwargs):
        super().__init__(*args, **kwargs)
        self._mask_center = bool(mask_center)
        kh, kw = self.weight.shape[2], self.weight.shape[3]
        mask = torch.zeros_like(self.weight)
        mask[:, :, : kh // 2, :] = 1.0
        mask[:, :, kh // 2, : kw // 2 + (0 if self._mask_center else 1)] = 1.0
        self.register_buffer("mask", mask)

    def _active_taps(self):
        m = self.mask[0, 0].detach().to("cpu")
        return [(u, v) for u in range(m.shape[0]) for v in range(m.shape[1]) if m[u, v] != 0]

    def forward(self, x, *, crop=None, in_act=None, res=None, **kw):
        ops.mul_inplace_(self.weight.data, self.mask)
        return super().forward(x, crop=crop, in_act=in_act, res=res, **kw)


class GatedActivation(nn.Module):

    def __init__(self, activation_fn=torch.tanh):
        super().__init__()
        self._activation_fn = activation_fn
        if activation_fn is torch.tanh or isinstance(activation_fn, nn.Tanh):
            self._gate = ops.GATE_TANH
        elif isinstance(activation_fn, nn.Identity):
            self._gate = ops.GATE_IDENTITY
        else:
            raise ValueError(
                "GatedActivation on the HIP path supports torch.tanh and nn.Identity() only"
            )

    def forward(self, x, *, res=None):
        _, c, _, _ = x.shape
        assert c % 2 == 0, "x must have an even number of channels."
        return ops.gated_activation(x, self._gate, res)


class GatedConv(nn.Module):

    def __init__(self, in_channels, out_channels, kernel_size=1, padding=0, mask_center=None,
                 activation_fn=torch.tanh, bias=True):
        super().__init__()
        if mask_center is None:
            self.conv = Conv2d(in_channels, 2 * out_channels, kernel_size, padding=padding, bias=bias)
        else:
            self.conv = CausalConv2d(mask_center, in_channels, 2 * out_channels, kernel_size, padding=padding,
                                     bias=bias)
        self.gate = GatedActivation(activation_fn)

    def forward(self, x, *, crop=None, in_act=None, res=None):
        if self.conv.gate_ok(x, crop):
            return self.conv(x, crop=crop, in_act=in_act, gate=self.gate._gate, gate_res=res)
        return self.gate(self.conv(x, crop=crop, in_act=in_act), res=res)


class NCHWLayerNorm(nn.LayerNorm):

    def forward(self, x, *, skip=False):
        if len(self.normalized_shape) != 1 or not self.elementwise_affine:
            raise ValueError("NCHWLayerNorm expects a single affine channel dimension")
        if skip and not ops.FUSE_LNSKIP:
            return ops.nchw_layernorm(x, self.weight, self.bias, self.eps), x
        if skip:
            return ops.nchw_layernorm_skip(x, self.weight, self.bias, self.eps)
        return ops.nchw_layernorm(x, self.weight, self.bias, self.eps)
```

### pytorch-generative_amd/pytorch_generative_amd/ops/__init__.py

```python

from pytorch_generative_amd.ops._common import (
    ACT_NONE,
    ACT_RELU,
    ACT_ELU,
    ACT_GELU,
    ACT_ELU_OUT,
    GATE_TANH,
    GATE_IDENTITY,
    _ACT_IDS,
    _stream,
    RowDecode,
    _chk,
    _p,
    zeros,
    zeros_like,
    _sink,
    CONV_FMT_F32,
    CONV_FMT_B3,
    CONV_FMT_B3_GATE,
    FUSE_SKIP,
    _dense_per_image,
)
from pytorch_generative_amd.ops.elementwise import (
    _ConcatChannels,
    concat_channels,
    _Act,
    relu,
    elu,
    gelu,
    _Gated,
    gated_activation,
    _Add,
    add,
    _AddBcast,
    add_broadcast_batch,
    image_positional_encoding,
    mul_inplace_,
    _sum_into,
    _SumVectors,
    _Fanout,
    fanout,
    sum_vectors,
)
from pytorch_generative_amd.ops.conv import (
    ConvSpec,
    CONV_MFMA,
    _use_mfma,
    _pack_frag,
    _pack_frag_both,
    _pack,
    _ConvTaps,
    FUSE_PAIR,
    FUSE_LNSKIP,
    FUSE_QKV_EXTRA,
    _adjacent_view,
    conv_pair_views,
    _ConvPair,
    conv2d_pair,
    conv_mfma_ok,
    conv_two_residuals_ok,
    conv2d_taps,
    conv_gate_ok,
    conv_dual_ok,
    GradSlot,
    FUSE_DUAL,
    FUSE_GATE,
)
from pytorch_generative_amd.ops.gpt_block import (
    FUSE_MLP,
    mlp_gelu_supported,
    _MlpGelu,
    mlp_gelu,
    FUSE_BLOCK,
    DEFER_BLOCK_REDUCE,
    _grad_targets,
    new_block_chain,
    assert_no_pending_block_reductions,
    flush_block_reductions,
    _GPTBlockHead,
    _GPTBlockTail,
    gpt_block_supported,
    gpt_block_head,
    gpt_block_tail,
    _NCHWLayerNorm,
    nchw_layernorm,
    nchw_layernorm_skip,
)
from pytorch_generative_amd.ops.attention import (
    _CausalAttention,
    _CausalAttentionQKV,
    _MergeQKVWeight,
    merge_qkv_weight,
    set_deterministic,
    causal_attention_qkv,
    attention_dims_native,
    _pad16,
    causal_attention,
)
from pytorch_generative_amd.ops.linear_attention import (
    _LinearCausalAttention,
    FEATURE_IDENTITY,
    FEATURE_ELU1,
    linear_causal_attention,
)
from pytorch_generative_amd.ops.masked_linear import (
    _MaskedMLP,
    mask_from_degrees,
    masked_linear,
    masked_mlp,
    mul_mask_,
)
from pytorch_generative_amd.ops.density import (
    _MixtureLogProb,
    MIXTURE_BERNOULLI,
    MIXTURE_GAUSSIAN,
    kde_gaussian,
    kde_parzen,
    mixture_log_prob,
)
from pytorch_generative_amd.ops.losses import (
    _BCEWithLogitsSumMean,
    _DmolLossSumMean,
    dmol_loss_sum_mean,
    DMOL_SAMPLE_MAX_K,
    dmol_sample,
    bce_with_logits_sum_mean,
    _ElboMean,
    elbo_terms,
)
from pytorch_generative_amd.ops.vae import (
    _AvgPool2,
    avg_pool2,
    _Upsample2,
    upsample2_nearest,
    _GaussHead,
    gaussian_head_unit,
    gaussian_head_pair,
    gaussian_head_prior,
    _PhaseSplit,
    _PhaseMerge,
    _PhaseWeights,
    _SplitInChannels,
    split_in_channels,
    phase_weights,
    phase_split,
    phase_merge,
    _PhaseMerge4,
    _PhaseSplit4,
    phase_split4,
    phase_merge4,
    _ConcatElu,
    concat_elu,
    _Resample2,
    subsample2,
    zero_insert2,
    col_subsample2,
    col_zero_insert2,
)
```

### pytorch-generative_amd/pytorch_generative_amd/ops/gpt_block.py

```python

import os

import torch

from pytorch_generative_amd import _lib
from pytorch_generative_amd.ops._common import _chk, _p, _sink, _stream, zeros, zeros_like


FUSE_MLP = os.environ.get("PG_FUSE_MLP", "1") != "0"


def mlp_gelu_supported(x, conv1, conv2):
    if not FUSE_MLP or conv1.bias is None or conv2.bias is None:
        return False
    w1, w2 = conv1.weight, conv2.weight
    return (tuple(w1.shape) == (64, 16, 1, 1) and tuple(w2.shape) == (16, 64, 1, 1)
            and x.shape[1] == 16 and (x.shape[2] * x.shape[3]) % 16 == 0)


class _MlpGelu(torch.autograd.Function):
    @staticmethod
    def forward(ctx, x, w1, b1, w2, b2, res, sinks):
        lib = _lib.load()
        x = _chk(x, "mlp_gelu.x")
        w1, b1, w2, b2 = (_chk(t, "mlp_gelu.param") for t in (w1, b1, w2, b2))
        if res is not None:
            res = _chk(res, "mlp_gelu.res")
        n, c, h, w = x.shape
        y = torch.empty_like(x)
        _lib.check(
            lib.pg_mlp_gelu_fwd(x.data_ptr(), w1.data_ptr(), b1.data_ptr(), w2.data_ptr(),
                                b2.data_ptr(), _p(res), y.data_ptr(), n, c, w1.shape[0], h * w,
                                _stream()),
            "pg_mlp_gelu_fwd",
        )
        ctx.save_for_backward(x, w1, b1, w2)
        ctx.sinks, ctx.has_res = sinks, res is not None
        return y

    @staticmethod
    def backward(ctx, dy):
        lib = _lib.load()
        x, w1, b1, w2 = ctx.saved_tensors
        dy = _chk(dy, "mlp_gelu.dy")
        n, c, h, w = x.shape
        hd = w1.shape[0]
        dx = torch.empty_like(x)
        grads, outs = [], []
        for sink, like in zip(ctx.sinks, (w1, b1, w2, None)):
            if sink is not None:
                grads.append(sink)
                outs.append(None)
            else:
                t = zeros((c,), x.device) if like is None else zeros_like(like)
                grads.append(t)
                outs.append(t)
        ws_n = lib.pg_mlp_gelu_bwd_workspace_floats(n, h * w)
        ws = torch.empty(ws_n, device=x.device, dtype=torch.float32)
        _lib.check(
            lib.pg_mlp_gelu_bwd(x.data_ptr(), w1.data_ptr(), b1.data_ptr(), w2.data_ptr(),
                                dy.data_ptr(), dx.data_ptr(), grads[0].data_ptr(),
                                grads[1].data_ptr(), grads[2].data_ptr(), grads[3].data_ptr(), n, c,
                                hd, h * w, ws.data_ptr(), ws_n, _stream()),
            "pg_mlp_gelu_bwd",
        )
        return dx, outs[0], outs[1], outs[2], outs[3], (dy if ctx.has_res else None), None


def mlp_gelu(x, conv1, conv2, res=None):
    sinks = (_sink(conv1.weight), _sink(conv1.bias), _sink(conv2.weight), _sink(conv2.bias))
    return _MlpGelu.apply(x, conv1.weight, conv1.bias, conv2.weight, conv2.bias, res, sinks)


FUSE_BLOCK = os.environ.get("PG_FUSE_BLOCK", "1") != "0"
DEFER_BLOCK_REDUCE = os.environ.get("PG_BLOCK_REDUCE_MERGED", "1") != "0"


def _grad_targets(params):
    tgt, ret = [], []
    for p in params:
        sink = _sink(p)
        if sink is not None:
            tgt.append(sink)
            ret.append(None)
        else:
            z = zeros_like(p)
            tgt.append(z)
            ret.append(z)
    return tgt, ret


_open_chains = []


def new_block_chain():
    import weakref

    class _Chain(dict):
        pass

    chain = _Chain(jobs=[])
    _open_chains[:] = [r for r in _open_chains if r() is not None]
    _open_chains.append(weakref.ref(chain))
    return chain


def assert_no_pending_block_reductions():
    for r in _open_chains:
        c = r()
        if c is not None and c["jobs"]:
            raise RuntimeError(f"{len(c['jobs'])} deferred GPT-block weight-gradient reductions were never flushed: the first "
                               "block's backward did not run (set PG_BLOCK_REDUCE_MERGED=0 to reduce per block)")


def flush_block_reductions(chain, n, c, L):
    import ctypes

    lib = _lib.load()
    jobs = chain["jobs"]
    for i in range(0, len(jobs), 8):
        grp = jobs[i:i + 8]
        hw = (ctypes.c_void_p * len(grp))(*[j[0].data_ptr() for j in grp])
        tw = (ctypes.c_void_p * len(grp))(*[j[1].data_ptr() for j in grp])
        gr = (ctypes.c_void_p * (14 * len(grp)))(*[ptr for j in grp for ptr in j[2]])
        _lib.check(lib.pg_gpt_blocks_reduce(len(grp), hw, tw, gr, n, c, L, _stream()), "pg_gpt_blocks_reduce")
    jobs.clear()


class _GPTBlockHead(torch.autograd.Function):

    @staticmethod
    def forward(ctx, x, lnw, lnb, wq, bq, wkv, bkv, eps, params, pair=None):
        lib = _lib.load()
        ctx.pair = pair
        x_in = x
        x = _chk(x, "gpt_block_head.x")
        n, c, h, w = x.shape
        qkv = torch.empty((n, 3 * c, h, w), device=x.device, dtype=torch.float32)
        _lib.check(
            lib.pg_gpt_block_head_fwd(x.data_ptr(), lnw.data_ptr(), lnb.data_ptr(), wq.data_ptr(),
                                      bq.data_ptr(), wkv.data_ptr(), bkv.data_ptr(), qkv.data_ptr(),
                                      n, c, h * w, eps, _stream()),
            "pg_gpt_block_head_fwd",
        )
        ctx.save_for_backward(x, lnw, lnb, wq, wkv)
        ctx.eps, ctx.params = eps, params
        return qkv, x_in

    @staticmethod
    def backward(ctx, dqkv, gx):
        lib = _lib.load()
        x, lnw, lnb, wq, wkv = ctx.saved_tensors
        n, c, h, w = x.shape
        pending = ctx.pair.pop("tail", None) if ctx.pair is not None else None
        if dqkv is None:
            if pending is not None:
                raise RuntimeError("gpt_block_head: a deferred tail reduction is pending but the head has no gradient")
            return gx, None, None, None, None, None, None, None, None, None
        dqkv = _chk(dqkv, "gpt_block_head.dqkv")
        gx = zeros_like(x) if gx is None else _chk(gx, "gpt_block_head.gx")
        dx = torch.empty_like(x)
        tgt, ret = _grad_targets(ctx.params)
        ws_n = lib.pg_gpt_block_head_bwd_workspace_floats(n, h * w)
        ws = torch.empty(ws_n, device=x.device, dtype=torch.float32)
        head_args = (x.data_ptr(), lnw.data_ptr(), lnb.data_ptr(), wq.data_ptr(),
                     wkv.data_ptr(), dqkv.data_ptr(), gx.data_ptr(), dx.data_ptr(),
                     tgt[0].data_ptr(), tgt[1].data_ptr(), tgt[2].data_ptr(),
                     tgt[3].data_ptr(), tgt[4].data_ptr(), tgt[5].data_ptr(), n, c,
                     h * w, ctx.eps, ws.data_ptr(), ws_n)
        chain = ctx.pair.get("chain") if ctx.pair is not None else None
        if pending is not None and chain is not None and all(r is None for r in ret):
            t_ws, t = pending
            _lib.check(lib.pg_gpt_block_head_bwd_partial(*head_args[:8], *head_args[14:], _stream()),
                       "pg_gpt_block_head_bwd_partial")
            chain["jobs"].append((ws, t_ws, [g.data_ptr() for g in tgt] + [t[4].data_ptr(), t[5].data_ptr(), t[6].data_ptr(),
                                                                          t[7].data_ptr(), t[0].data_ptr(), t[1].data_ptr(),
                                                                          t[2].data_ptr(), t[3].data_ptr()], (tgt, t)))
            if ctx.pair.get("flush"):
                flush_block_reductions(chain, n, c, h * w)
            return (dx, *ret, None, None, None)
        if pending is not None:
            t_ws, t = pending
            _lib.check(
                lib.pg_gpt_block_head_bwd_with_tail(*head_args, t_ws.data_ptr(), t[4].data_ptr(), t[5].data_ptr(),
                                                    t[6].data_ptr(), t[7].data_ptr(), t[0].data_ptr(),
                                                    t[1].data_ptr(), t[2].data_ptr(), t[3].data_ptr(), _stream()),
                "pg_gpt_block_head_bwd_with_tail",
            )
        else:
            _lib.check(lib.pg_gpt_block_head_bwd(*head_args, _stream()), "pg_gpt_block_head_bwd")
        return (dx, *ret, None, None, None)


class _GPTBlockTail(torch.autograd.Function):

    @staticmethod
    def forward(ctx, o, x, wp, bp, lnw, lnb, w1, b1, w2, b2, eps, params, pair=None):
        lib = _lib.load()
        ctx.pair = pair
        o = _chk(o, "gpt_block_tail.o")
        x = _chk(x, "gpt_block_tail.x")
        n, c, h, w = x.shape
        x_new = torch.empty_like(x)
        _lib.check(
            lib.pg_gpt_block_tail_fwd(o.data_ptr(), x.data_ptr(), wp.data_ptr(), bp.data_ptr(),
                                      lnw.data_ptr(), lnb.data_ptr(), w1.data_ptr(), b1.data_ptr(),
                                      w2.data_ptr(), b2.data_ptr(), x_new.data_ptr(), n, c,
                                      w1.shape[0], h * w, eps, _stream()),
            "pg_gpt_block_tail_fwd",
        )
        ctx.save_for_backward(o, x, wp, bp, lnw, lnb, w1, b1, w2)
        ctx.eps, ctx.params = eps, params
        return x_new

    @staticmethod
    def backward(ctx, d):
        lib = _lib.load()
        o, x, wp, bp, lnw, lnb, w1, b1, w2 = ctx.saved_tensors
        d = _chk(d, "gpt_block_tail.dx_new")
        n, c, h, w = x.shape
        d_o, gx = torch.empty_like(o), torch.empty_like(x)
        tgt, ret = _grad_targets(ctx.params)
        ws_n = lib.pg_gpt_block_tail_bwd_workspace_floats(n, h * w)
        ws = torch.empty(ws_n, device=x.device, dtype=torch.float32)
        if ctx.pair is not None and DEFER_BLOCK_REDUCE and all(r is None for r in ret):
            _lib.check(
                lib.pg_gpt_block_tail_bwd_partial(o.data_ptr(), x.data_ptr(), wp.data_ptr(), bp.data_ptr(),
                                                  lnw.data_ptr(), lnb.data_ptr(), w1.data_ptr(), b1.data_ptr(),
                                                  w2.data_ptr(), d.data_ptr(), d_o.data_ptr(), gx.data_ptr(), n, c,
                                                  w1.shape[0], h * w, ctx.eps, ws.data_ptr(), ws_n, _stream()),
                "pg_gpt_block_tail_bwd_partial",
            )
            ctx.pair["tail"] = (ws, tgt)
            return (d_o, gx, *ret, None, None, None)
        _lib.check(
            lib.pg_gpt_block_tail_bwd(o.data_ptr(), x.data_ptr(), wp.data_ptr(), bp.data_ptr(),
                                      lnw.data_ptr(), lnb.data_ptr(), w1.data_ptr(), b1.data_ptr(),
                                      w2.data_ptr(), d.data_ptr(), d_o.data_ptr(), gx.data_ptr(),
                                      tgt[0].data_ptr(), tgt[1].data_ptr(), tgt[2].data_ptr(),
                                      tgt[3].data_ptr(), tgt[4].data_ptr(), tgt[5].data_ptr(),
                                      tgt[6].data_ptr(), tgt[7].data_ptr(), n, c, w1.shape[0], h * w,
                                      ctx.eps, ws.data_ptr(), ws_n, _stream()),
            "pg_gpt_block_tail_bwd",
        )
        return (d_o, gx, *ret, None, None, None)


def gpt_block_supported(x, ln1, q, kv, proj, ln2, fc1, fc2):
    if not FUSE_BLOCK or x.shape[1] != 16 or (x.shape[2] * x.shape[3]) % 16 != 0:
        return False
    shapes = (tuple(q.weight.shape), tuple(kv.weight.shape), tuple(proj.weight.shape),
              tuple(fc1.weight.shape), tuple(fc2.weight.shape))
    if shapes != ((16, 16, 1, 1), (32, 16, 1, 1), (16, 16, 1, 1), (64, 16, 1, 1), (16, 64, 1, 1)):
        return False
    if any(m.bias is None for m in (q, kv, proj, fc1, fc2)):
        return False
    return tuple(ln1.normalized_shape) == (16,) and tuple(ln2.normalized_shape) == (16,)


def gpt_block_head(x, ln1, q, kv, pair=None):
    params = (ln1.weight, ln1.bias, q.weight, q.bias, kv.weight, kv.bias)
    return _GPTBlockHead.apply(x, *params, float(ln1.eps), params, pair)


def gpt_block_tail(o, x, proj, ln2, fc1, fc2, pair=None):
    params = (proj.weight, proj.bias, ln2.weight, ln2.bias, fc1.weight, fc1.bias, fc2.weight, fc2.bias)
    return _GPTBlockTail.apply(o, x, *params, float(ln2.eps), params, pair)


class _NCHWLayerNorm(torch.autograd.Function):
    @staticmethod
    def forward(ctx, x, gamma, beta, eps, gg, gb, with_skip=False):
        lib = _lib.load()
        x_in = x
        x = _chk(x, "layernorm.x")
        n, c, h, w = x.shape
        if gamma.numel() != c:
            raise ValueError(f"NCHWLayerNorm: normalized_shape {gamma.numel()} != channels {c}")
        y = torch.empty_like(x)
        mean = torch.empty(n * h * w, device=x.device, dtype=torch.float32)
        rstd = torch.empty_like(mean)
        _lib.check(
            lib.pg_nchw_layernorm_fwd(x.data_ptr(), gamma.data_ptr(), beta.data_ptr(), y.data_ptr(),
                                      mean.data_ptr(), rstd.data_ptr(), n, c, h * w, eps, _stream()),
            "pg_nchw_layernorm_fwd",
        )
        ctx.save_for_backward(x, gamma, mean, rstd)
        ctx.gg, ctx.gb = gg, gb
        if with_skip:
            return y, x_in
        return y

    @staticmethod
    def backward(ctx, dy, dskip=None):
        lib = _lib.load()
        x, gamma, mean, rstd = ctx.saved_tensors
        if dy is None:
            return dskip, None, None, None, None, None, None
        dy = _chk(dy, "layernorm.dy")
        n, c, h, w = x.shape
        dx = torch.empty_like(x)
        dg = db = None
        gg, gb = ctx.gg, ctx.gb
        if gg is None:
            dg = zeros((c,), x.device)
            gg = dg
        if gb is None:
            db = zeros((c,), x.device)
            gb = db
        ws_n = lib.pg_nchw_layernorm_bwd_workspace_floats(n, c, h * w)
        ws = torch.empty(ws_n, device=x.device, dtype=torch.float32)
        if dskip is None:
            _lib.check(
                lib.pg_nchw_layernorm_bwd(x.data_ptr(), gamma.data_ptr(), mean.data_ptr(),
                                          rstd.data_ptr(), dy.data_ptr(), dx.data_ptr(), gg.data_ptr(),
                                          gb.data_ptr(), n, c, h * w, ws.data_ptr(), ws_n, _stream()),
                "pg_nchw_layernorm_bwd",
            )
        else:
            dskip = _chk(dskip, "layernorm.dskip")
            _lib.check(
                lib.pg_nchw_layernorm_bwd_res(x.data_ptr(), gamma.data_ptr(), mean.data_ptr(),
                                              rstd.data_ptr(), dy.data_ptr(), dskip.data_ptr(),
                                              dx.data_ptr(), gg.data_ptr(), gb.data_ptr(), n, c,
                                              h * w, ws.data_ptr(), ws_n, _stream()),
                "pg_nchw_layernorm_bwd_res",
            )
        return dx, dg, db, None, None, None, None


def nchw_layernorm(x, weight, bias, eps=1e-5):
    return _NCHWLayerNorm.apply(x, weight, bias, float(eps), _sink(weight), _sink(bias))


def nchw_layernorm_skip(x, weight, bias, eps=1e-5):
    return _NCHWLayerNorm.apply(x, weight, bias, float(eps), _sink(weight), _sink(bias), True)
```

Before: 104,800 images/s.

## Fuse ImageGPT stem and output head into kernels with merged model-wide gradient reduction

Adds fused HIP kernels for the input stem (image plus positional embedding, then the masked 3x3 conv) and the output head (LayerNorm plus 1x1 conv), forward and backward. Their weight-gradient partials are folded into a single model-wide segmented reduction launch together with the transformer block reductions. The stem kernels exploit the centre-masked conv by computing only the four active taps and zeroing the masked weights. This is meant to cut kernel launches and intermediate memory traffic at both ends of the model. In exchange it adds specialised code paths gated on shape checks and an environment flag, which enlarges the surface for correctness bugs.

```diff
diff --git a/include/pg_hip.h b/include/pg_hip.h
--- a/include/pg_hip.h
+++ b/include/pg_hip.h
@@ -293,6 +293,23 @@
 int pg_broadcast(void* buf, size_t n, int dtype, int root, void* stream);
 int pg_comm_destroy(void);
 
+int pg_gpt_stem_fwd(const float* img, const float* pos, float* weight, const float* bias, float* x0, int N, int H, int W,
+                    int grid_cap, void* stream);
+int pg_gpt_stem_bwd_plan(int N, int H, int W, int grid_cap, int* rows, int* slices);
+size_t pg_gpt_stem_bwd_workspace_floats(int N, int H, int W, int grid_cap);
+int pg_gpt_stem_bwd(const float* dx0, const float* img, const float* pos, const float* weight, int N, int H, int W,
+                    int grid_cap, float* workspace, size_t workspace_floats, void* stream);
+int pg_gpt_out_head_fwd(const float* x, const float* ln_w, const float* ln_b, const float* conv_w, const float* conv_b,
+                        float* logits, int N, int C, int Cout, int L, float eps, int grid_cap, void* stream);
+int pg_gpt_out_head_bwd_rows(int N, int L, int grid_cap);
+int pg_gpt_out_head_bwd(const float* x, const float* ln_w, const float* ln_b, const float* conv_w, const float* dlogits,
+                        float* dx, int N, int C, int Cout, int L, float eps, int grid_cap, float* workspace,
+                        size_t workspace_floats, void* stream);
+int pg_gpt_model_reduce(int n_blocks, const float* const* head_ws, const float* const* tail_ws, float* const* grads, int N,
+                        int C, int L, const float* out_ws, int out_rows, int Cout, float* const* out_grads,
+                        const float* stem_ws, int stem_rows, int stem_slices, int H, int W, float* const* stem_grads,
+                        void* stream);
+
 #ifdef __cplusplus
 }
 #endif
diff --git a/pytorch-generative_amd/csrc/gpt_block.hip b/pytorch-generative_amd/csrc/gpt_block.hip
--- a/pytorch-generative_amd/csrc/gpt_block.hip
+++ b/pytorch-generative_amd/csrc/gpt_block.hip
@@ -1,6 +1,7 @@
 #include <stdlib.h>
 
 #include "common.h"
+#include "gpt_ends.h"
 
 namespace {
 
@@ -585,6 +586,52 @@
   red[rg][sl] = a0 + a1;
   __syncthreads();
   if (rg != 0 || s >= a.stride) return;
+  float acc = 0.f;
+#pragma unroll
+  for (int r = 0; r < 32; ++r) acc += red[r][sl];
+  int begin = 0;
+  for (int k = 0; k < a.nseg; ++k) {
+    if (s < a.end[k]) { a.dst[k][s - begin] += acc; return; }
+    begin = a.end[k];
+  }
+}
+
+constexpr int SEGM_MAX_JOBS = SEG_MAX_JOBS + 3;
+struct SegArgsM { SegArgs j[SEGM_MAX_JOBS]; int first[SEGM_MAX_JOBS + 1]; int n, pos_job, H, W; };
+__global__ void __launch_bounds__(256) seg_reduceM_kernel(const SegArgsM an) {
+  __shared__ float red[32][9];
+  int job = 0;
+  while (job + 1 < an.n && (int)blockIdx.x >= an.first[job + 1]) ++job;
+  const SegArgs& a = an.j[job];
+  const int blk = blockIdx.x - an.first[job];
+  const int sl = threadIdx.x & 7, rg = threadIdx.x >> 3;
+  const int s = blk * 8 + sl;
+  const int ncol = a.end[a.nseg - 1];
+  int col[4] = {s, -1, -1, -1};
+  if (job == an.pos_job && s < ncol) {
+    const int L = an.H * an.W, r = s / an.W, c = s - r * an.W;
+    col[0] = (r + 1 < an.H && c + 1 < an.W) ? 0 * L + s + an.W + 1 : -1;
+    col[1] = (r + 1 < an.H) ? 1 * L + s + an.W : -1;
+    col[2] = (r + 1 < an.H && c >= 1) ? 2 * L + s + an.W - 1 : -1;
+    col[3] = (c + 1 < an.W) ? 3 * L + s + 1 : -1;
+  }
+  float a0 = 0.f, a1 = 0.f;
+  if (s < ncol) {
+#pragma unroll
+    for (int k = 0; k < 4; ++k) {
+      if (col[k] < 0) continue;
+      const float* p = a.part + col[k];
+      int r = rg;
+      for (; r + 32 < a.rows; r += 64) {
+        a0 += p[(size_t)r * a.stride];
+        a1 += p[(size_t)(r + 32) * a.stride];
+      }
+      if (r < a.rows) a0 += p[(size_t)r * a.stride];
+    }
+  }
+  red[rg][sl] = a0 + a1;
+  __syncthreads();
+  if (rg != 0 || s >= ncol) return;
   float acc = 0.f;
 #pragma unroll
   for (int r = 0; r < 32; ++r) acc += red[r][sl];
@@ -774,6 +821,62 @@
   an.first[an.n] = nb;
   hipLaunchKernelGGL(seg_reduceN_kernel, dim3((unsigned)nb), dim3(256), 0, (hipStream_t)stream, an);
   PG_LAUNCH_CHECK("pg_gpt_blocks_reduce");
+  return 0;
+}
+
+PG_EXPORT int pg_gpt_model_reduce(int n_blocks, const float* const* head_ws, const float* const* tail_ws, float* const* grads,
+                                  int N, int Cc, int L, const float* out_ws, int out_rows, int Cout, float* const* out_grads,
+                                  const float* stem_ws, int stem_rows, int stem_slices, int H, int W,
+                                  float* const* stem_grads, void* stream) {
+  PG_REQUIRE(n_blocks >= 0 && 2 * n_blocks <= SEG_MAX_JOBS, PG_ESHAPE, "pg_gpt_model_reduce: 0..8 blocks per launch, got %d", n_blocks);
+  PG_REQUIRE(n_blocks == 0 || (head_ws && tail_ws && grads), PG_EINVAL, "pg_gpt_model_reduce: null pointer");
+  PG_REQUIRE(n_blocks > 0 || out_ws || stem_ws, PG_EINVAL, "pg_gpt_model_reduce: nothing to reduce");
+  if (n_blocks > 0)
+    if (int rc = check_shape("pg_gpt_model_reduce", N, Cc, L)) return rc;
+  SegArgsM an = {};
+  an.pos_job = -1;
+  int nb = 0, nj = 0;
+  for (int b = 0; b < n_blocks; ++b) {
+    float* const* g = grads + 14 * b;
+    PG_REQUIRE(head_ws[b] && tail_ws[b], PG_EINVAL, "pg_gpt_model_reduce: null workspace of block %d", b);
+    for (int k = 0; k < 14; ++k) PG_REQUIRE(g[k], PG_EINVAL, "pg_gpt_model_reduce: null gradient %d of block %d", k, b);
+    an.j[nj] = head_seg_args(head_ws[b], grid_blocks(1, N, L), g[0], g[1], g[2], g[3], g[4], g[5]);
+    an.first[nj++] = nb; nb += (H_PART + 7) / 8;
+    an.j[nj] = tail_seg_args(tail_ws[b], bwd_blocks(N, L), g[6], g[7], g[8], g[9], g[10], g[11], g[12], g[13]);
+    an.first[nj++] = nb; nb += (T_PART + 7) / 8;
+  }
+  if (out_ws) {
+    PG_REQUIRE(out_rows >= 1 && Cout >= 1 && Cout <= pg_ends::MAX_COUT && out_grads && out_grads[0] && out_grads[1] &&
+                   out_grads[2] && out_grads[3], PG_EINVAL, "pg_gpt_model_reduce: bad output-head arguments");
+    SegArgs r = {};
+    r.part = out_ws; r.rows = out_rows; r.stride = pg_ends::out_row_floats(Cout); r.nseg = 4;
+    r.end[0] = pg_ends::O_BE; r.dst[0] = out_grads[0];
+    r.end[1] = pg_ends::O_W; r.dst[1] = out_grads[1];
+    r.end[2] = pg_ends::O_W + Cout * pg_ends::C; r.dst[2] = out_grads[2];
+    r.end[3] = r.stride; r.dst[3] = out_grads[3];
+    an.j[nj] = r;
+    an.first[nj++] = nb; nb += (r.stride + 7) / 8;
+  }
+  if (stem_ws) {
+    PG_REQUIRE(stem_rows >= 1 && stem_slices >= 1 && H >= 1 && W >= 1 && stem_grads && stem_grads[0] && stem_grads[1] &&
+                   stem_grads[2], PG_EINVAL, "pg_gpt_model_reduce: bad stem arguments");
+    SegArgs r = {};
+    r.part = stem_ws; r.rows = stem_rows; r.stride = pg_ends::S_PART; r.nseg = 2;
+    r.end[0] = pg_ends::S_B; r.dst[0] = stem_grads[0];
+    r.end[1] = pg_ends::S_PART; r.dst[1] = stem_grads[1];
+    an.j[nj] = r;
+    an.first[nj++] = nb; nb += (pg_ends::S_PART + 7) / 8;
+    SegArgs q = {};
+    q.part = stem_ws + (size_t)stem_rows * pg_ends::S_PART; q.rows = stem_slices; q.stride = pg_ends::ACTIVE * H * W; q.nseg = 1;
+    q.end[0] = H * W; q.dst[0] = stem_grads[2];
+    an.pos_job = nj; an.H = H; an.W = W;
+    an.j[nj] = q;
+    an.first[nj++] = nb; nb += (H * W + 7) / 8;
+  }
+  an.n = nj;
+  an.first[nj] = nb;
+  hipLaunchKernelGGL(seg_reduceM_kernel, dim3((unsigned)nb), dim3(256), 0, (hipStream_t)stream, an);
+  PG_LAUNCH_CHECK("pg_gpt_model_reduce");
   return 0;
 }
 
diff --git a/pytorch-generative_amd/csrc/gpt_ends.h b/pytorch-generative_amd/csrc/gpt_ends.h
--- /dev/null
+++ b/pytorch-generative_amd/csrc/gpt_ends.h
@@ -0,0 +1,15 @@
+#pragma once
+
+namespace pg_ends {
+
+constexpr int C = 16;
+constexpr int MAX_COUT = 4;
+constexpr int TAPS = 9, ACTIVE = 4;
+
+constexpr int O_G = 0, O_BE = O_G + C, O_W = O_BE + C;
+constexpr int out_row_floats(int cout) { return O_W + cout * C + cout; }
+
+constexpr int S_W = 0, S_B = S_W + C * TAPS, S_PART = S_B + C;
+constexpr int stem_workspace_floats(int rows, int slices, int L) { return rows * S_PART + slices * ACTIVE * L; }
+
+}
diff --git a/pytorch-generative_amd/csrc/gpt_ends.hip b/pytorch-generative_amd/csrc/gpt_ends.hip
--- /dev/null
+++ b/pytorch-generative_amd/csrc/gpt_ends.hip
@@ -0,0 +1,499 @@
+#include "common.h"
+#include "gpt_ends.h"
+
+namespace {
+
+using namespace pg_ends;
+
+constexpr int THREADS = 256;
+constexpr int TILE_PX = 4 * THREADS;
+constexpr float INV_C = 1.f / 16.f;
+
+__device__ __forceinline__ float wave_sum(float s) {
+#pragma unroll
+  for (int m = 32; m >= 1; m >>= 1) s += __shfl_xor(s, m, 64);
+  return s;
+}
+
+template <int VEC>
+struct Px4 {
+  size_t img_off[4];
+  int p[4];
+  bool ok[4];
+  __device__ __forceinline__ Px4(long tile, long total, int L) {
+    if (VEC == 4) {
+      const long px = tile * TILE_PX + (long)threadIdx.x * 4;
+      const bool in = px < total;
+      const long n = in ? px / L : 0;
+      const int p0 = in ? (int)(px - n * L) : 0;
+#pragma unroll
+      for (int v = 0; v < 4; ++v) { ok[v] = in; p[v] = p0 + (in ? v : 0); img_off[v] = (size_t)n * L + p[v]; }
+      return;
+    }
+#pragma unroll
+    for (int v = 0; v < 4; ++v) {
+      const long px = tile * TILE_PX + (long)v * THREADS + threadIdx.x;
+      ok[v] = px < total;
+      const long n = ok[v] ? px / L : 0;
+      p[v] = ok[v] ? (int)(px - n * L) : 0;
+      img_off[v] = (size_t)n * L + p[v];
+    }
+  }
+  __device__ __forceinline__ size_t off(int v, int chans, int L) const { return (img_off[v] - p[v]) * chans + p[v]; }
+};
+
+template <int VEC>
+__device__ __forceinline__ void load_row(const float* __restrict__ t, const Px4<VEC>& q, int chans, int ch, int L, float out[4]) {
+  if (VEC == 4) {
+    if (q.ok[0]) {
+      const float4 f = *reinterpret_cast<const float4*>(t + q.off(0, chans, L) + (size_t)ch * L);
+      out[0] = f.x; out[1] = f.y; out[2] = f.z; out[3] = f.w;
+    } else {
+      out[0] = out[1] = out[2] = out[3] = 0.f;
+    }
+  } else {
+#pragma unroll
+    for (int v = 0; v < 4; ++v) out[v] = q.ok[v] ? t[q.off(v, chans, L) + (size_t)ch * L] : 0.f;
+  }
+}
+template <int VEC>
+__device__ __forceinline__ void store_row(float* __restrict__ t, const Px4<VEC>& q, int chans, int ch, int L, const float in[4]) {
+  if (VEC == 4) {
+    if (q.ok[0]) *reinterpret_cast<float4*>(t + q.off(0, chans, L) + (size_t)ch * L) = make_float4(in[0], in[1], in[2], in[3]);
+  } else {
+#pragma unroll
+    for (int v = 0; v < 4; ++v)
+      if (q.ok[v]) t[q.off(v, chans, L) + (size_t)ch * L] = in[v];
+  }
+}
+
+struct StemArgs {
+  const float* img; const float* pos; const float* w; const float* b; float* wmut; float* x0;
+  const float* dx0; float* part;
+  int N, H, W, L;
+  long total; int tiles;
+  int nchunks, chunk_px, slices, btiles;
+};
+
+__device__ __forceinline__ float stem_in(const StemArgs& a, size_t img_base, int r, int c) {
+  if (r < 0 || r >= a.H || c < 0 || c >= a.W) return 0.f;
+  const int o = r * a.W + c;
+  return a.img[img_base + o] + a.pos[o];
+}
+
+template <int VEC>
+__global__ void __launch_bounds__(THREADS) stem_fwd_kernel(const StemArgs a) {
+  float w[C][ACTIVE], bb[C];
+#pragma unroll
+  for (int ch = 0; ch < C; ++ch) {
+    bb[ch] = a.b[ch];
+#pragma unroll
+    for (int t = 0; t < ACTIVE; ++t) w[ch][t] = a.w[ch * TAPS + t];
+  }
+  for (long tile = blockIdx.x; tile < a.tiles; tile += gridDim.x) {
+    const Px4<VEC> q(tile, a.total, a.L);
+    float in[ACTIVE][4];
+#pragma unroll
+    for (int v = 0; v < 4; ++v) {
+      const int r = q.p[v] / a.W, c = q.p[v] - r * a.W;
+      const size_t base = q.img_off[v] - q.p[v];
+      in[0][v] = q.ok[v] ? stem_in(a, base, r - 1, c - 1) : 0.f;
+      in[1][v] = q.ok[v] ? stem_in(a, base, r - 1, c) : 0.f;
+      in[2][v] = q.ok[v] ? stem_in(a, base, r - 1, c + 1) : 0.f;
+      in[3][v] = q.ok[v] ? stem_in(a, base, r, c - 1) : 0.f;
+    }
+#pragma unroll
+    for (int ch = 0; ch < C; ++ch) {
+      float out[4];
+#pragma unroll
+      for (int v = 0; v < 4; ++v)
+        out[v] = fmaf(w[ch][3], in[3][v], fmaf(w[ch][2], in[2][v], fmaf(w[ch][1], in[1][v], fmaf(w[ch][0], in[0][v], bb[ch]))));
+      store_row<VEC>(a.x0, q, C, ch, a.L, out);
+    }
+  }
+  if (blockIdx.x == 0 && threadIdx.x < C * (TAPS - ACTIVE))
+    a.wmut[(threadIdx.x / (TAPS - ACTIVE)) * TAPS + ACTIVE + threadIdx.x % (TAPS - ACTIVE)] = 0.f;
+}
+
+constexpr int SB_PX = 128, SB_CH = 8;
+__global__ void __launch_bounds__(THREADS) stem_bwd_kernel(const StemArgs a) {
+  __shared__ float gs[2][ACTIVE][SB_PX];
+  __shared__ float red[4][SB_CH * (TAPS + 1)];
+  const int lane = threadIdx.x & 63, wv = threadIdx.x >> 6;
+  const int cg = wv & 1, q = (wv >> 1) * 64 + lane;
+  const int L = a.L;
+  float aw[SB_CH][TAPS], ab[SB_CH];
+#pragma unroll
+  for (int cc = 0; cc < SB_CH; ++cc) {
+    ab[cc] = 0.f;
+#pragma unroll
+    for (int t = 0; t < TAPS; ++t) aw[cc][t] = 0.f;
+  }
+  float* part_b = a.part + (size_t)gridDim.x * S_PART;
+  for (int tile = blockIdx.x; tile < a.btiles; tile += gridDim.x) {
+    const int k = tile % a.nchunks, s = tile / a.nchunks;
+    const int start = k * a.chunk_px;
+    const int p = start + q;
+    const bool ok = q < a.chunk_px && p < L;
+    const int r = p / a.W, c = p - r * a.W;
+    int off[TAPS];
+    bool valid[TAPS];
+#pragma unroll
+    for (int t = 0; t < TAPS; ++t) {
+      const int rr = r + t / 3 - 1, cc = c + t % 3 - 1;
+      valid[t] = ok && rr >= 0 && rr < a.H && cc >= 0 && cc < a.W;
+      off[t] = valid[t] ? rr * a.W + cc : (ok ? p : 0);
+    }
+    const float* dbase = a.dx0 + (size_t)(SB_CH * cg) * L + (ok ? p : 0);
+    auto load_d = [&](int n, float d[SB_CH]) {
+      const float* b = dbase + (size_t)n * C * L;
+#pragma unroll
+      for (int cc = 0; cc < SB_CH; ++cc) d[cc] = ok ? b[(size_t)cc * L] : 0.f;
+    };
+    float D[SB_CH], d[SB_CH], dn[SB_CH];
+#pragma unroll
+    for (int cc = 0; cc < SB_CH; ++cc) D[cc] = 0.f;
+    load_d(s, d);
+    for (int n = s; n < a.N; n += a.slices) {
+      const int nn = n + a.slices;
+      load_d(nn < a.N ? nn : n, dn);
+      const float* im = a.img + (size_t)n * L;
+      float in[TAPS];
+#pragma unroll
+      for (int t = 0; t < TAPS; ++t) {
+        const float x = im[off[t]];
+        in[t] = valid[t] ? x : 0.f;
+      }
+#pragma unroll
+      for (int cc = 0; cc < SB_CH; ++cc) {
+        D[cc] += d[cc];
+#pragma unroll
+        for (int t = 0; t < TAPS; ++t) aw[cc][t] = fmaf(d[cc], in[t], aw[cc][t]);
+        d[cc] = dn[cc];
+      }
+    }
+    float G[ACTIVE] = {0.f, 0.f, 0.f, 0.f};
+#pragma unroll
+    for (int t = 0; t < TAPS; ++t) {
+      const float x = a.pos[off[t]];
+      const float pv = valid[t] ? x : 0.f;
+#pragma unroll
+      for (int cc = 0; cc < SB_CH; ++cc) aw[cc][t] = fmaf(D[cc], pv, aw[cc][t]);
+    }
+#pragma unroll
+    for (int cc = 0; cc < SB_CH; ++cc) {
+      ab[cc] += D[cc];
+#pragma unroll
+      for (int t = 0; t < ACTIVE; ++t) G[t] = fmaf(a.w[(SB_CH * cg + cc) * TAPS + t], D[cc], G[t]);
+    }
+#pragma unroll
+    for (int t = 0; t < ACTIVE; ++t) gs[cg][t][q] = G[t];
+    __syncthreads();
+    for (int i = threadIdx.x; i < ACTIVE * SB_PX; i += THREADS) {
+      const int t = i / SB_PX, qq = i % SB_PX;
+      if (qq < a.chunk_px && start + qq < L) part_b[((size_t)s * ACTIVE + t) * L + start + qq] = gs[0][t][qq] + gs[1][t][qq];
+    }
+    __syncthreads();
+  }
+#pragma unroll
+  for (int cc = 0; cc < SB_CH; ++cc) {
+#pragma unroll
+    for (int t = 0; t < TAPS; ++t) {
+      const float v = wave_sum(aw[cc][t]);
+      if (lane == 0) red[wv][cc * TAPS + t] = v;
+    }
+    const float v = wave_sum(ab[cc]);
+    if (lane == 0) red[wv][SB_CH * TAPS + cc] = v;
+  }
+  __syncthreads();
+  float* row = a.part + (size_t)blockIdx.x * S_PART;
+  if (threadIdx.x < 2 * SB_CH * (TAPS + 1)) {
+    const int g = threadIdx.x / (SB_CH * (TAPS + 1)), j = threadIdx.x % (SB_CH * (TAPS + 1));
+    const float v = red[g][j] + red[g + 2][j];
+    if (j < SB_CH * TAPS) row[S_W + SB_CH * TAPS * g + j] = v;
+    else row[S_B + SB_CH * g + (j - SB_CH * TAPS)] = v;
+  }
+}
+
+struct OutArgs {
+  const float* x; const float* g; const float* be; const float* cw; const float* cb; float* logits;
+  const float* dl; float* dx; float* part;
+  int N, L; long total; int tiles; float eps;
+};
+
+__device__ __forceinline__ float ln_normalise(float x[C], float eps) {
+  float s = 0.f;
+#pragma unroll
+  for (int c = 0; c < C; ++c) s += x[c];
+  const float mu = s * INV_C;
+  float q = 0.f;
+#pragma unroll
+  for (int c = 0; c < C; ++c) { x[c] -= mu; q = fmaf(x[c], x[c], q); }
+  const float var = q * INV_C + eps;
+  float rs = rsqrtf(var);
+  rs = rs * (1.5f - 0.5f * var * rs * rs);
+#pragma unroll
+  for (int c = 0; c < C; ++c) x[c] *= rs;
+  return rs;
+}
+
+template <int VEC, int COUT>
+__global__ void __launch_bounds__(THREADS) out_fwd_kernel(const OutArgs a) {
+  float g[C], be[C], cw[COUT][C];
+#pragma unroll
+  for (int c = 0; c < C; ++c) {
+    g[c] = a.g[c]; be[c] = a.be[c];
+#pragma unroll
+    for (int co = 0; co < COUT; ++co) cw[co][c] = a.cw[co * C + c];
+  }
+  float cb[COUT];
+#pragma unroll
+  for (int co = 0; co < COUT; ++co) cb[co] = a.cb[co];
+  for (long tile = blockIdx.x; tile < a.tiles; tile += gridDim.x) {
+    const Px4<VEC> q(tile, a.total, a.L);
+    float x[C][4];
+#pragma unroll
+    for (int c = 0; c < C; ++c) load_row<VEC>(a.x, q, C, c, a.L, x[c]);
+    float out[COUT][4];
+#pragma unroll
+    for (int v = 0; v < 4; ++v) {
+      float xv[C];
+#pragma unroll
+      for (int c = 0; c < C; ++c) xv[c] = x[c][v];
+      ln_normalise(xv, a.eps);
+#pragma unroll
+      for (int c = 0; c < C; ++c) xv[c] = fmaf(xv[c], g[c], be[c]);
+#pragma unroll
+      for (int co = 0; co < COUT; ++co) {
+        float o = cb[co];
+#pragma unroll
+        for (int c = 0; c < C; ++c) o = fmaf(cw[co][c], xv[c], o);
+        out[co][v] = o;
+      }
+    }
+#pragma unroll
+    for (int co = 0; co < COUT; ++co) store_row<VEC>(a.logits, q, COUT, co, a.L, out[co]);
+  }
+}
+
+template <int VEC, int COUT>
+__global__ void __launch_bounds__(THREADS) out_bwd_kernel(const OutArgs a) {
+  __shared__ float red[4][COUT * (C + 1)];
+  float g[C], be[C], cw[COUT][C];
+#pragma unroll
+  for (int c = 0; c < C; ++c) {
+    g[c] = a.g[c]; be[c] = a.be[c];
+#pragma unroll
+    for (int co = 0; co < COUT; ++co) cw[co][c] = a.cw[co * C + c];
+  }
+  float S[COUT][C], T[COUT];
+#pragma unroll
+  for (int co = 0; co < COUT; ++co) {
+    T[co] = 0.f;
+#pragma unroll
+    for (int c = 0; c < C; ++c) S[co][c] = 0.f;
+  }
+  for (long tile = blockIdx.x; tile < a.tiles; tile += gridDim.x) {
+    const Px4<VEC> q(tile, a.total, a.L);
+    float x[C][4], dl[COUT][4];
+#pragma unroll
+    for (int c = 0; c < C; ++c) load_row<VEC>(a.x, q, C, c, a.L, x[c]);
+#pragma unroll
+    for (int co = 0; co < COUT; ++co) load_row<VEC>(a.dl, q, COUT, co, a.L, dl[co]);
+#pragma unroll
+    for (int v = 0; v < 4; ++v) {
+      float xh[C], dxh[C];
+#pragma unroll
+      for (int c = 0; c < C; ++c) xh[c] = x[c][v];
+      const float rs = ln_normalise(xh, a.eps);
+      float m1 = 0.f, m2 = 0.f;
+#pragma unroll
+      for (int c = 0; c < C; ++c) {
+        float dy = 0.f;
+#pragma unroll
+        for (int co = 0; co < COUT; ++co) dy = fmaf(cw[co][c], dl[co][v], dy);
+        dxh[c] = dy * g[c];
+        m1 += dxh[c];
+        m2 = fmaf(dxh[c], xh[c], m2);
+      }
+      m1 *= INV_C; m2 *= INV_C;
+#pragma unroll
+      for (int co = 0; co < COUT; ++co) {
+        T[co] += dl[co][v];
+#pragma unroll
+        for (int c = 0; c < C; ++c) S[co][c] = fmaf(dl[co][v], xh[c], S[co][c]);
+      }
+#pragma unroll
+      for (int c = 0; c < C; ++c) x[c][v] = rs * (dxh[c] - m1 - xh[c] * m2);
+    }
+#pragma unroll
+    for (int c = 0; c < C; ++c) store_row<VEC>(a.dx, q, C, c, a.L, x[c]);
+  }
+  const int lane = threadIdx.x & 63, wv = threadIdx.x >> 6;
+#pragma unroll
+  for (int co = 0; co < COUT; ++co) {
+#pragma unroll
+    for (int c = 0; c < C; ++c) {
+      const float v = wave_sum(S[co][c]);
+      if (lane == 0) red[wv][co * (C + 1) + c] = v;
+    }
+    const float v = wave_sum(T[co]);
+    if (lane == 0) red[wv][co * (C + 1) + C] = v;
+  }
+  __syncthreads();
+  float* row = a.part + (size_t)blockIdx.x * out_row_floats(COUT);
+  auto tot = [&](int i) { return (red[0][i] + red[1][i]) + (red[2][i] + red[3][i]); };
+  if (threadIdx.x < C) {
+    const int c = threadIdx.x;
+    float dg = 0.f, db = 0.f;
+#pragma unroll
+    for (int co = 0; co < COUT; ++co) {
+      const float s = tot(co * (C + 1) + c), t = tot(co * (C + 1) + C), w = a.cw[co * C + c];
+      dg = fmaf(w, s, dg);
+      db = fmaf(w, t, db);
+      row[O_W + co * C + c] = fmaf(a.g[c], s, a.be[c] * t);
+    }
+    row[O_G + c] = dg;
+    row[O_BE + c] = db;
+  } else if (threadIdx.x < C + COUT) {
+    const int co = threadIdx.x - C;
+    row[O_W + COUT * C + co] = tot(co * (C + 1) + C);
+  }
+}
+
+bool al16(const void* p) { return (reinterpret_cast<uintptr_t>(p) & 15) == 0; }
+
+int tile_grid(long total_px, int grid_cap, int* tiles) {
+  const long t = (total_px + TILE_PX - 1) / TILE_PX;
+  *tiles = (int)t;
+  const long cap = grid_cap > 0 ? grid_cap : 2048;
+  return (int)(t < cap ? t : cap);
+}
+
+struct StemPlan { int nchunks, chunk_px, slices, tiles, grid; };
+StemPlan stem_plan(int N, int L, int grid_cap) {
+  StemPlan p;
+  p.nchunks = (L + SB_PX - 1) / SB_PX;
+  p.chunk_px = (L + p.nchunks - 1) / p.nchunks;
+  int s = 512 / p.nchunks;
+  if (s < 1) s = 1;
+  p.slices = N < s ? N : s;
+  p.tiles = p.nchunks * p.slices;
+  const int cap = grid_cap > 0 ? grid_cap : 1024;
+  p.grid = p.tiles < cap ? p.tiles : cap;
+  return p;
+}
+
+int check_dims(const char* who, int N, long L) {
+  PG_REQUIRE(N > 0 && L > 0, PG_EINVAL, "%s: non-positive dimension", who);
+  PG_REQUIRE((long)N * L * C < (1L << 40) && L < (1L << 30), PG_ESHAPE, "%s: tensor too large", who);
+  return 0;
+}
+
+}
+
+PG_EXPORT int pg_gpt_stem_fwd(const float* img, const float* pos, float* weight, const float* bias, float* x0, int N,
+                              int H, int W, int grid_cap, void* stream) {
+  PG_REQUIRE(img && pos && weight && bias && x0, PG_EINVAL, "pg_gpt_stem_fwd: null pointer");
+  PG_REQUIRE(H > 0 && W > 0 && grid_cap >= 0, PG_EINVAL, "pg_gpt_stem_fwd: bad argument");
+  const long L = (long)H * W;
+  if (int rc = check_dims("pg_gpt_stem_fwd", N, L)) return rc;
+  StemArgs a = {};
+  a.img = img; a.pos = pos; a.w = weight; a.wmut = weight; a.b = bias; a.x0 = x0;
+  a.N = N; a.H = H; a.W = W; a.L = (int)L; a.total = (long)N * L;
+  const int grid = tile_grid(a.total, grid_cap, &a.tiles);
+  if (L % 4 == 0 && al16(x0))
+    hipLaunchKernelGGL(stem_fwd_kernel<4>, dim3((unsigned)grid), dim3(THREADS), 0, (hipStream_t)stream, a);
+  else
+    hipLaunchKernelGGL(stem_fwd_kernel<1>, dim3((unsigned)grid), dim3(THREADS), 0, (hipStream_t)stream, a);
+  PG_LAUNCH_CHECK("pg_gpt_stem_fwd");
+  return 0;
+}
+
+PG_EXPORT int pg_gpt_stem_bwd_plan(int N, int H, int W, int grid_cap, int* rows, int* slices) {
+  PG_REQUIRE(N > 0 && H > 0 && W > 0 && grid_cap >= 0 && rows && slices, PG_EINVAL, "pg_gpt_stem_bwd_plan: bad argument");
+  const StemPlan p = stem_plan(N, H * W, grid_cap);
+  *rows = p.grid; *slices = p.slices;
+  return 0;
+}
+PG_EXPORT size_t pg_gpt_stem_bwd_workspace_floats(int N, int H, int W, int grid_cap) {
+  if (N <= 0 || H <= 0 || W <= 0 || grid_cap < 0) return 0;
+  const StemPlan p = stem_plan(N, H * W, grid_cap);
+  return (size_t)stem_workspace_floats(p.grid, p.slices, H * W);
+}
+
+PG_EXPORT int pg_gpt_stem_bwd(const float* dx0, const float* img, const float* pos, const float* weight, int N, int H,
+                              int W, int grid_cap, float* workspace, size_t workspace_floats, void* stream) {
+  PG_REQUIRE(dx0 && img && pos && weight && workspace, PG_EINVAL, "pg_gpt_stem_bwd: null pointer");
+  PG_REQUIRE(H > 0 && W > 0 && grid_cap >= 0, PG_EINVAL, "pg_gpt_stem_bwd: bad argument");
+  const long L = (long)H * W;
+  if (int rc = check_dims("pg_gpt_stem_bwd", N, L)) return rc;
+  PG_REQUIRE(workspace_floats >= pg_gpt_stem_bwd_workspace_floats(N, H, W, grid_cap), PG_EINVAL,
+             "pg_gpt_stem_bwd: workspace too small");
+  const StemPlan p = stem_plan(N, (int)L, grid_cap);
+  StemArgs a = {};
+  a.dx0 = dx0; a.img = img; a.pos = pos; a.w = weight; a.part = workspace;
+  a.N = N; a.H = H; a.W = W; a.L = (int)L;
+  a.nchunks = p.nchunks; a.chunk_px = p.chunk_px; a.slices = p.slices; a.btiles = p.tiles;
+  hipLaunchKernelGGL(stem_bwd_kernel, dim3((unsigned)p.grid), dim3(THREADS), 0, (hipStream_t)stream, a);
+  PG_LAUNCH_CHECK("pg_gpt_stem_bwd");
+  return 0;
+}
+
+namespace {
+template <int VEC>
+int launch_out(bool bwd, int cout, int grid, hipStream_t st, const OutArgs& a) {
+#define PG_OUT_CASE(K)                                                                                   \
+  case K:                                                                                                \
+    if (bwd) hipLaunchKernelGGL((out_bwd_kernel<VEC, K>), dim3((unsigned)grid), dim3(THREADS), 0, st, a); \
+    else hipLaunchKernelGGL((out_fwd_kernel<VEC, K>), dim3((unsigned)grid), dim3(THREADS), 0, st, a);     \
+    return 0;
+  switch (cout) {
+    PG_OUT_CASE(1) PG_OUT_CASE(2) PG_OUT_CASE(3) PG_OUT_CASE(4)
+  }
+#undef PG_OUT_CASE
+  return PG_ESHAPE;
+}
+}
+
+PG_EXPORT int pg_gpt_out_head_fwd(const float* x, const float* ln_w, const float* ln_b, const float* conv_w,
+                                  const float* conv_b, float* logits, int N, int Cc, int Cout, int L, float eps,
+                                  int grid_cap, void* stream) {
+  PG_REQUIRE(x && ln_w && ln_b && conv_w && conv_b && logits && grid_cap >= 0, PG_EINVAL, "pg_gpt_out_head_fwd: bad argument");
+  PG_REQUIRE(Cc == C, PG_ESHAPE, "pg_gpt_out_head_fwd: only C = 16 is instantiated (got %d)", Cc);
+  PG_REQUIRE(Cout >= 1 && Cout <= MAX_COUT, PG_ESHAPE, "pg_gpt_out_head_fwd: 1..%d output channels (got %d)", MAX_COUT, Cout);
+  if (int rc = check_dims("pg_gpt_out_head_fwd", N, L)) return rc;
+  OutArgs a = {};
+  a.x = x; a.g = ln_w; a.be = ln_b; a.cw = conv_w; a.cb = conv_b; a.logits = logits;
+  a.N = N; a.L = L; a.total = (long)N * L; a.eps = eps;
+  const int grid = tile_grid(a.total, grid_cap, &a.tiles);
+  if (L % 4 == 0 && al16(x) && al16(logits)) launch_out<4>(false, Cout, grid, (hipStream_t)stream, a);
+  else launch_out<1>(false, Cout, grid, (hipStream_t)stream, a);
+  PG_LAUNCH_CHECK("pg_gpt_out_head_fwd");
+  return 0;
+}
+
+PG_EXPORT int pg_gpt_out_head_bwd_rows(int N, int L, int grid_cap) {
+  if (N <= 0 || L <= 0 || grid_cap < 0) return 0;
+  int tiles;
+  return tile_grid((long)N * L, grid_cap, &tiles);
+}
+
+PG_EXPORT int pg_gpt_out_head_bwd(const float* x, const float* ln_w, const float* ln_b, const float* conv_w,
+                                  const float* dlogits, float* dx, int N, int Cc, int Cout, int L, float eps, int grid_cap,
+                                  float* workspace, size_t workspace_floats, void* stream) {
+  PG_REQUIRE(x && ln_w && ln_b && conv_w && dlogits && dx && workspace && grid_cap >= 0, PG_EINVAL,
+             "pg_gpt_out_head_bwd: bad argument");
+  PG_REQUIRE(Cc == C, PG_ESHAPE, "pg_gpt_out_head_bwd: only C = 16 is instantiated (got %d)", Cc);
+  PG_REQUIRE(Cout >= 1 && Cout <= MAX_COUT, PG_ESHAPE, "pg_gpt_out_head_bwd: 1..%d output channels (got %d)", MAX_COUT, Cout);
+  if (int rc = check_dims("pg_gpt_out_head_bwd", N, L)) return rc;
+  OutArgs a = {};
+  a.x = x; a.g = ln_w; a.be = ln_b; a.cw = conv_w; a.dl = dlogits; a.dx = dx; a.part = workspace;
+  a.N = N; a.L = L; a.total = (long)N * L; a.eps = eps;
+  const int grid = tile_grid(a.total, grid_cap, &a.tiles);
+  PG_REQUIRE(workspace_floats >= (size_t)grid * out_row_floats(Cout), PG_EINVAL, "pg_gpt_out_head_bwd: workspace too small");
+  if (L % 4 == 0 && al16(x) && al16(dlogits) && al16(dx)) launch_out<4>(true, Cout, grid, (hipStream_t)stream, a);
+  else launch_out<1>(true, Cout, grid, (hipStream_t)stream, a);
+  PG_LAUNCH_CHECK("pg_gpt_out_head_bwd");
+  return 0;
+}
diff --git a/pytorch-generative_amd/pytorch_generative_amd/_lib.py b/pytorch-generative_amd/pytorch_generative_amd/_lib.py
--- a/pytorch-generative_amd/pytorch_generative_amd/_lib.py
+++ b/pytorch-generative_amd/pytorch_generative_amd/_lib.py
@@ -60,6 +60,17 @@
     "pg_gpt_block_head_bwd_partial": (c_i, [c_f] * 8 + [c_i, c_i, c_i, c_flt, c_f, c_z, c_s]),
     "pg_gpt_blocks_reduce": (c_i, [c_i, ctypes.POINTER(ctypes.c_void_p), ctypes.POINTER(ctypes.c_void_p),
                                    ctypes.POINTER(ctypes.c_void_p), c_i, c_i, c_i, c_s]),
+    "pg_gpt_stem_fwd": (c_i, [c_f] * 5 + [c_i, c_i, c_i, c_i, c_s]),
+    "pg_gpt_stem_bwd_plan": (c_i, [c_i, c_i, c_i, c_i, c_ip, c_ip]),
+    "pg_gpt_stem_bwd_workspace_floats": (c_z, [c_i, c_i, c_i, c_i]),
+    "pg_gpt_stem_bwd": (c_i, [c_f] * 4 + [c_i, c_i, c_i, c_i, c_f, c_z, c_s]),
+    "pg_gpt_out_head_fwd": (c_i, [c_f] * 6 + [c_i, c_i, c_i, c_i, c_flt, c_i, c_s]),
+    "pg_gpt_out_head_bwd_rows": (c_i, [c_i, c_i, c_i]),
+    "pg_gpt_out_head_bwd": (c_i, [c_f] * 6 + [c_i, c_i, c_i, c_i, c_flt, c_i, c_f, c_z, c_s]),
+    "pg_gpt_model_reduce": (c_i, [c_i, ctypes.POINTER(ctypes.c_void_p), ctypes.POINTER(ctypes.c_void_p),
+                                  ctypes.POINTER(ctypes.c_void_p), c_i, c_i, c_i, c_f, c_i, c_i,
+                                  ctypes.POINTER(ctypes.c_void_p), c_f, c_i, c_i, c_i, c_i,
+                                  ctypes.POINTER(ctypes.c_void_p), c_s]),
     "pg_gpt_block_tail_fwd": (c_i, [c_f] * 11 + [c_i, c_i, c_i, c_i, c_flt, c_s]),
     "pg_gpt_block_tail_bwd": (c_i, [c_f] * 20 + [c_i, c_i, c_i, c_i, c_flt, c_f, c_z, c_s]),
     "pg_gpt_block_tail_bwd_workspace_floats": (c_z, [c_i, c_i]),
diff --git a/pytorch-generative_amd/pytorch_generative_amd/models/autoregressive/image_gpt.py b/pytorch-generative_amd/pytorch_generative_amd/models/autoregressive/image_gpt.py
--- a/pytorch-generative_amd/pytorch_generative_amd/models/autoregressive/image_gpt.py
+++ b/pytorch-generative_amd/pytorch_generative_amd/models/autoregressive/image_gpt.py
@@ -167,14 +167,26 @@
         return canvas
 
     def forward(self, x):
-        x = self._input(ops.add_broadcast_batch(x, self._pos))
-        blocks = list(self._transformer)
+        img, blocks, grad = x, list(self._transformer), torch.is_grad_enabled()
+        fuse_stem = ops.gpt_stem_supported(img, self._pos, self._input)
+        stem_flushes = fuse_stem and grad and any(p.requires_grad for p in (self._pos, self._input.weight, self._input.bias))
+        if fuse_stem:
+            x0_grad = stem_flushes
+            probe = torch.empty(1, self._input.weight.shape[0], img.shape[2], img.shape[3], device="meta")
+        else:
+            x = probe = self._input(ops.add_broadcast_batch(img, self._pos))
+            x0_grad = x.requires_grad
         chain = None
-        if (ops.DEFER_BLOCK_REDUCE and _BLOCK_CHAIN and torch.is_grad_enabled() and x.requires_grad and len(blocks) > 1
-                and all(b._fused_ok(x) for b in blocks)):
+        if (ops.DEFER_BLOCK_REDUCE and _BLOCK_CHAIN and grad and x0_grad and len(blocks) > 1
+                and all(b._fused_ok(probe) for b in blocks)
+                and (stem_flushes or all(ops._sink(p) is not None for b in blocks for p in b.parameters()))):
             chain = ops.new_block_chain()
+        if fuse_stem:
+            x = self._input(img, pos=self._pos, chain=chain if stem_flushes else None)
         for i, block in enumerate(blocks):
-            x = block.forward_plus_input(x, chain, flush=(i == 0))
+            x = block.forward_plus_input(x, chain, flush=(i == 0 and not stem_flushes))
+        if ops.gpt_out_head_supported(x, self._ln, self._out):
+            return self._out(x, pre_ln=self._ln, chain=chain if stem_flushes else None)
         return self._out(self._ln(x))
 
 
diff --git a/pytorch-generative_amd/pytorch_generative_amd/nn/convolution.py b/pytorch-generative_amd/pytorch_generative_amd/nn/convolution.py
--- a/pytorch-generative_amd/pytorch_generative_amd/nn/convolution.py
+++ b/pytorch-generative_amd/pytorch_generative_amd/nn/convolution.py
@@ -100,7 +100,14 @@
                 and ops.conv_dual_ok(x, self.weight, self._conv_spec()))
 
     def forward(self, x, *, crop=None, in_act=None, res=None, out_act=None, out_pre_scaled=False,
-                in_post=None, n_skip=0, res2=None, gate=None, gate_res=None, res_slot=None, in_sum=None):
+                in_post=None, n_skip=0, res2=None, gate=None, gate_res=None, res_slot=None, in_sum=None, pre_ln=None,
+                chain=None):
+        if pre_ln is not None:
+            if (crop is not None or in_act is not None or res is not None or out_act is not None or n_skip or res2 is not None
+                    or gate is not None or res_slot is not None or in_sum is not None or ops.RowDecode.current is not None
+                    or not ops.gpt_out_head_supported(x, pre_ln, self)):
+                raise ValueError("Conv2d: pre_ln= needs a plain 1x1 convolution on a shape gpt_out_head_supported() accepts")
+            return ops.gpt_out_head(x, pre_ln, self, chain)
         if res_slot is not None or in_sum is not None:
             if (gate is not None or res2 is not None or n_skip or self._down2 or ops.RowDecode.current is not None
                     or not self.mfma_ok(x, crop)):
@@ -215,7 +222,12 @@
         m = self.mask[0, 0].detach().to("cpu")
         return [(u, v) for u in range(m.shape[0]) for v in range(m.shape[1]) if m[u, v] != 0]
 
-    def forward(self, x, *, crop=None, in_act=None, res=None, **kw):
+    def forward(self, x, *, crop=None, in_act=None, res=None, pos=None, chain=None, **kw):
+        if pos is not None:
+            if (crop is not None or in_act is not None or res is not None or kw or ops.RowDecode.current is not None
+                    or not ops.gpt_stem_supported(x, pos, self)):
+                raise ValueError("CausalConv2d: pos= needs the plain stem shape gpt_stem_supported() accepts")
+            return ops.gpt_stem(x, pos, self, chain)
         ops.mul_inplace_(self.weight.data, self.mask)
         return super().forward(x, crop=crop, in_act=in_act, res=res, **kw)
 
diff --git a/pytorch-generative_amd/pytorch_generative_amd/ops/__init__.py b/pytorch-generative_amd/pytorch_generative_amd/ops/__init__.py
--- a/pytorch-generative_amd/pytorch_generative_amd/ops/__init__.py
+++ b/pytorch-generative_amd/pytorch_generative_amd/ops/__init__.py
@@ -86,6 +86,17 @@
     nchw_layernorm,
     nchw_layernorm_skip,
 )
+from pytorch_generative_amd.ops.gpt_ends import (
+    FUSE_ENDS,
+    model_reduce,
+    flush_model_reductions,
+    gpt_stem_supported,
+    _GPTStem,
+    gpt_stem,
+    gpt_out_head_supported,
+    _GPTOutHead,
+    gpt_out_head,
+)
 from pytorch_generative_amd.ops.attention import (
     _CausalAttention,
     _CausalAttentionQKV,
diff --git a/pytorch-generative_amd/pytorch_generative_amd/ops/gpt_block.py b/pytorch-generative_amd/pytorch_generative_amd/ops/gpt_block.py
--- a/pytorch-generative_amd/pytorch_generative_amd/ops/gpt_block.py
+++ b/pytorch-generative_amd/pytorch_generative_amd/ops/gpt_block.py
@@ -108,9 +108,10 @@
 def assert_no_pending_block_reductions():
     for r in _open_chains:
         c = r()
-        if c is not None and c["jobs"]:
-            raise RuntimeError(f"{len(c['jobs'])} deferred GPT-block weight-gradient reductions were never flushed: the first "
-                               "block's backward did not run (set PG_BLOCK_REDUCE_MERGED=0 to reduce per block)")
+        if c is not None and (c["jobs"] or c.get("out") is not None):
+            raise RuntimeError(f"{len(c['jobs']) + (c.get('out') is not None)} deferred ImageGPT weight-gradient reductions were "
+                               "never flushed: the backward that flushes them (the stem's, else the first block's) did not run "
+                               "(set PG_BLOCK_REDUCE_MERGED=0 to reduce per block)")
 
 
 def flush_block_reductions(chain, n, c, L):
@@ -153,7 +154,11 @@
         x, lnw, lnb, wq, wkv = ctx.saved_tensors
         n, c, h, w = x.shape
         pending = ctx.pair.pop("tail", None) if ctx.pair is not None else None
+        chain = ctx.pair.get("chain") if ctx.pair is not None else None
+        flusher = chain is not None and bool(ctx.pair.get("flush"))
         if dqkv is None:
+            if flusher and chain["jobs"]:
+                flush_block_reductions(chain, n, c, h * w)
             if pending is not None:
                 raise RuntimeError("gpt_block_head: a deferred tail reduction is pending but the head has no gradient")
             return gx, None, None, None, None, None, None, None, None, None
@@ -168,7 +173,6 @@
                      tgt[0].data_ptr(), tgt[1].data_ptr(), tgt[2].data_ptr(),
                      tgt[3].data_ptr(), tgt[4].data_ptr(), tgt[5].data_ptr(), n, c,
                      h * w, ctx.eps, ws.data_ptr(), ws_n)
-        chain = ctx.pair.get("chain") if ctx.pair is not None else None
         if pending is not None and chain is not None and all(r is None for r in ret):
             t_ws, t = pending
             _lib.check(lib.pg_gpt_block_head_bwd_partial(*head_args[:8], *head_args[14:], _stream()),
@@ -176,9 +180,11 @@
             chain["jobs"].append((ws, t_ws, [g.data_ptr() for g in tgt] + [t[4].data_ptr(), t[5].data_ptr(), t[6].data_ptr(),
                                                                           t[7].data_ptr(), t[0].data_ptr(), t[1].data_ptr(),
                                                                           t[2].data_ptr(), t[3].data_ptr()], (tgt, t)))
-            if ctx.pair.get("flush"):
+            if flusher:
                 flush_block_reductions(chain, n, c, h * w)
             return (dx, *ret, None, None, None)
+        if flusher and chain["jobs"]:
+            flush_block_reductions(chain, n, c, h * w)
         if pending is not None:
             t_ws, t = pending
             _lib.check(
diff --git a/pytorch-generative_amd/pytorch_generative_amd/ops/gpt_ends.py b/pytorch-generative_amd/pytorch_generative_amd/ops/gpt_ends.py
--- /dev/null
+++ b/pytorch-generative_amd/pytorch_generative_amd/ops/gpt_ends.py
@@ -0,0 +1,159 @@
+
+import ctypes
+import os
+
+import torch
+
+from pytorch_generative_amd import _lib
+from pytorch_generative_amd.ops._common import RowDecode, _chk, _stream
+from pytorch_generative_amd.ops.gpt_block import _grad_targets
+
+FUSE_ENDS = os.environ.get("PG_FUSE_ENDS", "1") != "0"
+MAX_OUT_CHANNELS = 4
+
+
+def _ptrs(tensors):
+    return (ctypes.c_void_p * len(tensors))(*[t.data_ptr() for t in tensors])
+
+
+def model_reduce(jobs, n, c, L, out=None, stem=None):
+    lib = _lib.load()
+    assert len(jobs) <= 8
+    hw = _ptrs([j[0] for j in jobs]) if jobs else None
+    tw = _ptrs([j[1] for j in jobs]) if jobs else None
+    gr = (ctypes.c_void_p * (14 * len(jobs)))(*[ptr for j in jobs for ptr in j[2]]) if jobs else None
+    o_ws, o_rows, o_cout, o_tgt = out if out is not None else (None, 0, 0, None)
+    s_ws, s_rows, s_slices, h, w, s_tgt = stem if stem is not None else (None, 0, 0, 0, 0, None)
+    _lib.check(
+        lib.pg_gpt_model_reduce(len(jobs), hw, tw, gr, n, c, L,
+                                0 if o_ws is None else o_ws.data_ptr(), o_rows, o_cout, None if o_tgt is None else _ptrs(o_tgt),
+                                0 if s_ws is None else s_ws.data_ptr(), s_rows, s_slices, h, w,
+                                None if s_tgt is None else _ptrs(s_tgt), _stream()),
+        "pg_gpt_model_reduce",
+    )
+
+
+def flush_model_reductions(chain, n, c, L, stem=None):
+    from pytorch_generative_amd.ops.gpt_block import flush_block_reductions
+
+    jobs = chain["jobs"]
+    out = chain.pop("out", None)
+    last = jobs[max(0, len(jobs) - 8):] if jobs else []
+    if len(jobs) > 8:
+        del jobs[len(jobs) - 8:]
+        flush_block_reductions(chain, n, c, L)
+    if last or out is not None or stem is not None:
+        model_reduce(last, n, c, L, out=out, stem=stem)
+    jobs.clear()
+
+
+def gpt_stem_supported(img, pos, conv):
+    if (not FUSE_ENDS or RowDecode.current is not None or conv.bias is None or not getattr(conv, "_mask_center", False)
+            or not hasattr(conv, "mask")):
+        return False
+    pad = conv.padding if isinstance(conv.padding, tuple) else (conv.padding, conv.padding)
+    stride = conv.stride if isinstance(conv.stride, tuple) else (conv.stride, conv.stride)
+    return (img.dim() == 4 and img.shape[1] == 1 and tuple(conv.weight.shape) == (16, 1, 3, 3) and tuple(pad) == (1, 1)
+            and tuple(stride) == (1, 1) and tuple(pos.shape) == (1, 1, img.shape[2], img.shape[3])
+            and not img.requires_grad and img.is_cuda and img.dtype == torch.float32)
+
+
+class _GPTStem(torch.autograd.Function):
+
+    @staticmethod
+    def forward(ctx, img, pos, weight, bias, params, chain, grid_cap):
+        lib = _lib.load()
+        img = _chk(img, "gpt_stem.img")
+        pos, weight, bias = (_chk(t, "gpt_stem.param") for t in (pos, weight, bias))
+        n, _, h, w = img.shape
+        x0 = torch.empty((n, 16, h, w), device=img.device, dtype=torch.float32)
+        _lib.check(lib.pg_gpt_stem_fwd(img.data_ptr(), pos.data_ptr(), weight.data_ptr(), bias.data_ptr(), x0.data_ptr(),
+                                       n, h, w, grid_cap, _stream()), "pg_gpt_stem_fwd")
+        ctx.save_for_backward(img, pos, weight)
+        ctx.params, ctx.chain, ctx.grid_cap = params, chain, grid_cap
+        return x0
+
+    @staticmethod
+    def backward(ctx, dx0):
+        lib = _lib.load()
+        img, pos, weight = ctx.saved_tensors
+        n, _, h, w = img.shape
+        chain = ctx.chain
+        try:
+            dx0 = _chk(dx0, "gpt_stem.dx0")
+            tgt, ret = _grad_targets(ctx.params)
+            rows, slices = ctypes.c_int(0), ctypes.c_int(0)
+            _lib.check(lib.pg_gpt_stem_bwd_plan(n, h, w, ctx.grid_cap, ctypes.byref(rows), ctypes.byref(slices)),
+                       "pg_gpt_stem_bwd_plan")
+            ws_n = lib.pg_gpt_stem_bwd_workspace_floats(n, h, w, ctx.grid_cap)
+            ws = torch.empty(ws_n, device=img.device, dtype=torch.float32)
+            _lib.check(lib.pg_gpt_stem_bwd(dx0.data_ptr(), img.data_ptr(), pos.data_ptr(), weight.data_ptr(), n, h, w,
+                                           ctx.grid_cap, ws.data_ptr(), ws_n, _stream()), "pg_gpt_stem_bwd")
+            stem = (ws, rows.value, slices.value, h, w, [tgt[1], tgt[2], tgt[0]])
+        except BaseException:
+            if chain is not None:
+                flush_model_reductions(chain, n, 16, h * w)
+            raise
+        if chain is not None:
+            flush_model_reductions(chain, n, 16, h * w, stem=stem)
+        else:
+            model_reduce([], n, 16, h * w, stem=stem)
+        return None, ret[0], ret[1], ret[2], None, None, None
+
+
+def gpt_stem(img, pos, conv, chain=None, grid_cap=0):
+    params = (pos, conv.weight, conv.bias)
+    return _GPTStem.apply(img, pos, conv.weight, conv.bias, params, chain, grid_cap)
+
+
+def gpt_out_head_supported(x, ln, conv):
+    if not FUSE_ENDS or RowDecode.current is not None or conv.bias is None or x.dim() != 4 or x.shape[1] != 16:
+        return False
+    cout = conv.weight.shape[0]
+    return (tuple(conv.weight.shape) == (cout, 16, 1, 1) and 1 <= cout <= MAX_OUT_CHANNELS
+            and tuple(ln.normalized_shape) == (16,) and type(conv).__name__ == "Conv2d")
+
+
+class _GPTOutHead(torch.autograd.Function):
+
+    @staticmethod
+    def forward(ctx, x, lnw, lnb, cw, cb, eps, params, chain, grid_cap):
+        lib = _lib.load()
+        x = _chk(x, "gpt_out_head.x")
+        lnw, lnb, cw, cb = (_chk(t, "gpt_out_head.param") for t in (lnw, lnb, cw, cb))
+        n, c, h, w = x.shape
+        cout = cw.shape[0]
+        logits = torch.empty((n, cout, h, w), device=x.device, dtype=torch.float32)
+        _lib.check(lib.pg_gpt_out_head_fwd(x.data_ptr(), lnw.data_ptr(), lnb.data_ptr(), cw.data_ptr(), cb.data_ptr(),
+                                           logits.data_ptr(), n, c, cout, h * w, eps, grid_cap, _stream()),
+                   "pg_gpt_out_head_fwd")
+        ctx.save_for_backward(x, lnw, lnb, cw)
+        ctx.eps, ctx.params, ctx.chain, ctx.grid_cap = eps, params, chain, grid_cap
+        return logits
+
+    @staticmethod
+    def backward(ctx, dlogits):
+        lib = _lib.load()
+        x, lnw, lnb, cw = ctx.saved_tensors
+        n, c, h, w = x.shape
+        cout, L = cw.shape[0], h * w
+        dlogits = _chk(dlogits, "gpt_out_head.dlogits")
+        dx = torch.empty_like(x)
+        tgt, ret = _grad_targets(ctx.params)
+        rows = lib.pg_gpt_out_head_bwd_rows(n, L, ctx.grid_cap)
+        ws_n = rows * (32 + 17 * cout)
+        ws = torch.empty(ws_n, device=x.device, dtype=torch.float32)
+        _lib.check(lib.pg_gpt_out_head_bwd(x.data_ptr(), lnw.data_ptr(), lnb.data_ptr(), cw.data_ptr(),
+                                           dlogits.data_ptr(), dx.data_ptr(), n, c, cout, L, ctx.eps, ctx.grid_cap,
+                                           ws.data_ptr(), ws_n, _stream()), "pg_gpt_out_head_bwd")
+        out = (ws, rows, cout, tgt)
+        if ctx.chain is not None and all(r is None for r in ret):
+            ctx.chain["out"] = out
+        else:
+            model_reduce([], n, c, L, out=out)
+        return dx, ret[0], ret[1], ret[2], ret[3], None, None, None, None
+
+
+def gpt_out_head(x, ln, conv, chain=None, grid_cap=0):
+    params = (ln.weight, ln.bias, conv.weight, conv.bias)
+    return _GPTOutHead.apply(x, *params, float(ln.eps), params, chain, grid_cap)
```

Result: faster. 107,200 images/s, median of 6 (+2.3%).
